# Makiato1999/HRI-EMO

Hardware: AMD Instinct MI355X
Metric: utterances/sec fwd+bwd, d=768 T_a=400 T_t=128 N_e=6 (higher is better)
Workload: dtype bf16; 1 GPU; FusionWithEmotionDecoder fwd+bwd (train mode, dropout 0.1), d=768 T_a=400 T_t=128 N_e=6 H=8, 2 fusion + 2 decoder layers, all-False masks (BASELINE cfg2); global_batch=64, batch_per_gpu=64, parallelism=dp1, grad_allreduce=none, launch=hipGraph replay, streams=2

## Files before the change

### hri-emo_amd/__init__.py

```python
from . import _lib
from .models.cross_modal_block_tacfn import CrossModalBlock, CrossModalTransformer
from .models.beta_gate_tacfn import BetaGate
from .models.emotion_decoder import EmotionDecoder, ExplainableDecoderLayer
from .models.fusion_with_emotion_decoder import FusionWithEmotionDecoder
from .models.mosei_fusion_with_emotion_decoder import MoseiFusionWithEmotionDecoder
from .models.fusion_classifier import FusionClassifier

from .dp import EvalStep
from ._ops import set_gemm_mode, gemm_mode, enable_fused_wgrad, set_precision, precision, set_varlen, varlen, set_varlen_maps, varlen_maps, set_mfma_maps, mfma_maps, set_ingest, ingest

__all__ = ["EvalStep", "set_gemm_mode", "gemm_mode", "enable_fused_wgrad", "set_precision", "precision", "set_varlen", "varlen", "set_varlen_maps", "varlen_maps", "set_mfma_maps", "mfma_maps", "set_ingest", "ingest", "CrossModalBlock", "CrossModalTransformer", "BetaGate", "EmotionDecoder", "ExplainableDecoderLayer",
           "FusionWithEmotionDecoder", "MoseiFusionWithEmotionDecoder", "FusionClassifier"]
```

### hri-emo_amd/_lib.py

```python
import ctypes
import os

_HERE = os.path.dirname(os.path.abspath(__file__))
LIB_PATH = os.environ.get("HRIEMO_LIB") or os.path.join(_HERE, "libhriemo.so")

_C = {"p": ctypes.c_void_p, "i": ctypes.c_int, "l": ctypes.c_long, "f": ctypes.c_float,
      "Q": ctypes.c_ulonglong, "I": ctypes.c_uint}

_SIGS = {
    "hriemo_gemm_bf16": ("iiiiiplplplipipliplp", "i"),
    "hriemo_gemm_force_config": ("i", "i"),
    "hriemo_gemm_debug_flags": ("i", "i"),
    "hriemo_gemm_colsum_rows": ("iiiii", "i"),
    "hriemo_gemm_plan": ("iiiiiilppp", "i"),
    "hriemo_gemm_bf16_group_tn": ("piip", "i"),
    "hriemo_gemm_bf16_split": ("iiiiiplplplpliiplp", "i"),
    "hriemo_gemm_bf16_colsum": ("iiiiiplplplplpp", "i"),
    "hriemo_mx8_scale_ld": ("i", "l"),
    "hriemo_quant_mx8": ("pliiiplplp", "i"),
    "hriemo_gemm_mx8": ("iiiplplplplplipiplp", "i"),
    "hriemo_gemm_mx8_q": ("iiiplplplplplpiplplp", "i"),
    "hriemo_gemm_mx8_force_config": ("i", "i"),
    "hriemo_attn_fwd": ("plplplplppiiiiifQpIipp", "i"),
    "hriemo_attn_fwd_q": ("plplplplppiiiiifQpIipplplp", "i"),
    "hriemo_attn_bwd": ("plplplplplplplplpppiiiiifQpIipppp", "i"),
    "hriemo_attn_fwd_varlen": ("plplplplpppiiiiifQpIipp", "i"),
    "hriemo_attn_fwd_q_varlen": ("plplplplpppiiiiifQpIipplpllp", "i"),
    "hriemo_attn_bwd_varlen": ("plplplplplplplplppppiiiiifQpIipppp", "i"),
    "hriemo_attn_mask_bytes": ("iiii", "l"),
    "hriemo_attn_bwd_single_pass": ("iiii", "i"),
    "hriemo_attn_bwd_single_pass_q": ("iiiii", "i"),
    "hriemo_attn_bwd_kv_colsum_rows": ("iiiii", "i"),
    "hriemo_attn_bwd_colsum_rows": ("iiii", "i"),
    "hriemo_attn_bwd_dq_colsum_rows": ("iiiii", "i"),
    "hriemo_attn_plan": ("iiiiiipppppp", "i"),
    "hriemo_split_bf16x3": ("pliipiip", "i"),
    "hriemo_attn_fwd_f32": ("plplplplppiiiiifQpIip", "i"),
    "hriemo_attn_probs_f32": ("plplpppiiiiifQpIip", "i"),
    "hriemo_add_ln_f32": ("ppppppiiffQpIlp", "i"),
    "hriemo_dropout_f32": ("ppliipfQpIlp", "i"),
    "hriemo_masked_mean_f32": ("pppiiip", "i"),
    "hriemo_gate_input_f32": ("pppiip", "i"),
    "hriemo_sigmoid_beta_f32": ("pppiip", "i"),
    "hriemo_fuse_f32": ("ppipippiiip", "i"),
    "hriemo_split3_f32": ("pliipiiplp", "i"),
    "hriemo_colsum_f32_workspace_bytes": ("ii", "l"),
    "hriemo_colsum_f32": ("pliiplpipp", "i"),
    "hriemo_add_ln_bwd_f32_workspace_bytes": ("ii", "l"),
    "hriemo_add_ln_bwd_f32": ("pppppppppiiiffQpIlpp", "i"),
    "hriemo_attn_bwd_f32": ("plplplplplppplplplpiiiiifQpIip", "i"),
    "hriemo_gate_dpre_f32": ("ppipipppiiip", "i"),
    "hriemo_gate_input_bwd_f32": ("pppppiip", "i"),
    "hriemo_gate_dy_f32": ("ppipppiiiip", "i"),
    "hriemo_rowdot_bwd_f32": ("ppppppiiip", "i"),
    "hriemo_attn_fwd_f32_varlen": ("plplplplpppiiiiifQpIip", "i"),
    "hriemo_attn_bwd_f32_varlen": ("plplplplplpppplplplpiiiiifQpIip", "i"),
    "hriemo_add_ln_f32_rows": ("ppppppiiffQpIlpp", "i"),
    "hriemo_add_ln_bwd_f32_rows": ("pppppppppiiiffQpIlppp", "i"),
    "hriemo_masked_mean_f32_packed": ("ppipiiip", "i"),
    "hriemo_fuse_f32_packed": ("pppiippiipppiiiip", "i"),
    "hriemo_gate_dpre_f32_packed": ("ppippiippiipppiiip", "i"),
    "hriemo_gate_dy_f32_packed": ("ppipippipiiiip", "i"),
    "hriemo_attn_probs": ("plplpppiiiiifQpIip", "i"),
    "hriemo_attn_probs_mfma": ("plplpppiiiiifQpIip", "i"),
    "hriemo_attn_probs_varlen": ("plplppppiiiiiiifQpIip", "i"),
    "hriemo_attn_probs_f32_varlen": ("plplppppiiiiiiifQpIip", "i"),
    "hriemo_add_ln_fwd": ("pppppppppiiffQpIlp", "i"),
    "hriemo_add_ln_fwd_mx8": ("pppppppppiiffQpIlpplp", "i"),
    "hriemo_add_ln_fwd_rows": ("pppppppppiiffQpIlpplpp", "i"),
    "hriemo_add_ln_bwd_rows": ("ppppppppppppiiifQpIlppp", "i"),
    "hriemo_add_ln_bwd_workspace_bytes": ("ii", "l"),
    "hriemo_add_ln_bwd": ("ppppppppppppiiifQpIlpp", "i"),
    "hriemo_colsum_workspace_bytes": ("ii", "l"),
    "hriemo_colsum_bf16": ("pliipipp", "i"),
    "hriemo_cast_f32_to_bf16": ("pplp", "i"),
    "hriemo_cast_bf16_to_f32": ("pplp", "i"),
    "hriemo_cast_f32_to_bf16_batch": ("pip", "i"),
    "hriemo_cast_copy_batch": ("pip", "i"),
    "hriemo_pack_rows": ("pppiiiipppp", "i"),
    "hriemo_unpack_rows": ("pppiiippp", "i"),
    "hriemo_ingest_rows": ("pilpiiiiipppplpp", "i"),
    "hriemo_seq_tables": ("ppiiiiippppppp", "i"),
    "hriemo_gather_rows": ("plppiplp", "i"),
    "hriemo_dropout_bf16": ("pplifQpIlp", "i"),
    "hriemo_gemm_ln_supported": ("i", "i"),
    "hriemo_gemm_ln_fwd": ("iiiplplppppppppppffQpIlpp", "i"),
    "hriemo_expand_rows": ("pppilp", "i"),
    "hriemo_seed_bump": ("pp", "i"),
    "hriemo_rowdot_fwd": ("pppppiip", "i"),
    "hriemo_rowdot_bwd": ("pppppppiiip", "i"),
    "hriemo_pool_chunks": ("i", "i"),
    "hriemo_ln_pool_fwd": ("pppppppppiiiifp", "i"),
    "hriemo_gate_input": ("ppppiiiipppp" + "p", "i"),
    "hriemo_sigmoid_beta": ("pppiip", "i"),
    "hriemo_fuse_fwd": ("ppppiiip", "i"),
    "hriemo_add_ln_bwd_partial_rows": ("ii", "i"),
    "hriemo_rowops_force_variant": ("i", "i"),
    "hriemo_colsum_partial_rows": ("ii", "i"),
    "hriemo_colreduce_batch": ("pipip", "i"),
    "hriemo_debug_hog": ("iipp", "i"),
    "hriemo_sumsq_f32": ("plpip", "i"),
    "hriemo_adamw_flat": ("pppplfffffifpp", "i"),
    "hriemo_optim_finalize": ("pippppp", "i"),
    "hriemo_adamw_flat_dev": ("pppplppp", "i"),
    "hriemo_grad_begin": ("plpp", "i"),
    "hriemo_optim_finalize_ctl": ("pipppppp", "i"),
    "hriemo_masked_mean_fwd": ("ppppiiip", "i"),
    "hriemo_rowsum_f32": ("ppilp", "i"),
    "hriemo_gate_input_pooled": ("pppiip", "i"),
    "hriemo_fusion_loss": ("ppppiiiffpppp", "i"),
    "hriemo_fusion_loss_ce": ("pppiiiffpppp", "i"),
    "hriemo_fusion_loss_n": ("ppppiiiffppppp", "i"),
    "hriemo_fusion_loss_ce_n": ("pppiiiffppppp", "i"),
    "hriemo_stats_update": ("ppppfpipiiippippp", "i"),
    "hriemo_predict_log": ("ppipiiipppipp", "i"),
    "hriemo_attn_log_plan": ("ppiipppp", "i"),
    "hriemo_attn_log_close": ("pp", "i"),
    "hriemo_attn_log_append": ("piippip", "i"),
    "hriemo_attn_probs_varlen_log": ("plplppppiiiiiiifQpIipip", "i"),
    "hriemo_attn_probs_varlen_log_fp32": ("plplppppiiiiiiifQpIipip", "i"),
    "hriemo_stats_counts": ("ppiippipp", "i"),
    "hriemo_stats_auc_tiles": ("i", "i"),
    "hriemo_stats_auc": ("ppiipppp", "i"),
    "hriemo_scalar_gate_dx":("pipippppiiip", "i"),
    "hriemo_fuse_bwd_dw": ("ppppiiip", "i"),
    "hriemo_gate_dpre": ("pippp" + "iip", "i"),
    "hriemo_gate_input_bwd": ("ppppppiip", "i"),
    "hriemo_ln_pool_bwd_chunks": ("i", "i"),
    "hriemo_ln_pool_pair_supported": ("i", "i"),
    "hriemo_ln_pool_fwd_pair": ("pppppppppi" * 2 + "iiifp", "i"),
    "hriemo_ln_pool_bwd_pair": ("pip" + "ppppppppppip" * 2 + "iiip", "i"),
    "hriemo_ln_pool_bwd_workspace_bytes": ("iii", "l"),
    "hriemo_ln_pool_bwd": ("pipipppppppppp" + "iiiipp", "i"),
    "hriemo_ln_pool_fwd_packed": ("pppiippppppipiiifp", "i"),
    "hriemo_ln_pool_fwd_packed_pair": ("pppiippppppi" * 2 + "piiifp", "i"),
    "hriemo_fuse_fwd_packed": ("pppppiiiip", "i"),
    "hriemo_fuse_fwd_packed_q": ("pppppiiiipplp", "i"),
    "hriemo_fuse_bwd_dw_packed": ("pppppiiiip", "i"),
    "hriemo_ln_pool_bwd_packed": ("ppipippppiipppppp" + "iiiipp", "i"),
    "hriemo_ln_pool_bwd_packed_pair": ("ppip" + "ppppiippppppip" * 2 + "iiip", "i"),
    "hriemo_prof_enable": ("i", "i"),
    "hriemo_prof_nclass": ("", "i"),
    "hriemo_prof_collect": ("ippp", "i"),
    "hriemo_abi_version": ("", "i"),
}

_lib = None


def lib():
    global _lib
    if _lib is None:
        if not os.path.exists(LIB_PATH):
            raise RuntimeError(
                f"{LIB_PATH} not found: build it with `make -C hri-emo_amd/csrc` (or __graft_entry__.build()). "
                "There is no CPU/eager fallback for this path.")
        L = ctypes.CDLL(LIB_PATH)
        for name, (args, res) in _SIGS.items():
            fn = getattr(L, name)
            fn.argtypes = [_C[c] for c in args]
            fn.restype = _C[res]
        L.hriemo_last_error.restype = ctypes.c_char_p
        L.hriemo_last_error.argtypes = []
        L.hriemo_prof_name.restype = ctypes.c_char_p
        L.hriemo_prof_name.argtypes = [ctypes.c_int]
        _lib = L
    return _lib


def call(name, *args):
    L = lib()
    rc = getattr(L, name)(*args)
    if rc != 0:
        raise RuntimeError(f"{name} failed ({rc}): {L.hriemo_last_error().decode()}")
```

### hri-emo_amd/_ops.py

```python
import itertools
import os as _os
import threading
from collections import namedtuple

import torch

from . import _lib

BF16 = torch.bfloat16
_EPS = 1e-5
_apply_tls = threading.local()


def _stream():
    return torch.cuda.current_stream().cuda_stream


def _p(t):
    return None if t is None else t.data_ptr()


def _require_fp32_master(p):
    if p.dtype != torch.float32:
        raise TypeError(f"hri_emo_amd: parameter of dtype {p.dtype}; keep the module's parameters in fp32 "
# ... 102 lines not shown
        t.record_stream(stream)
    return t


class TextBranch:

    def __init__(self, side, main):
        self.side, self.main = side, main

    def fork(self, *handed):
        if self.side is not None:
            fork(self.side, self.main)
            for x in handed:
                share(x, self.side)

    def run(self):
        return torch.cuda.stream(self.side)

    def join(self, *back):
        if self.side is not None:
            self.main.wait_stream(self.side)
            for x in back:
                share(x, self.main)


_site_counter = itertools.count(1)


def new_site_base():
    return next(_site_counter) * 4


_seed_words = {}
STEP_ID = 0


def begin_step():
    global STEP_ID
    STEP_ID += 1
    CTX.half_reports.clear()

WEIGHTS_EPOCH = 0


def bump_weights_epoch():
    global WEIGHTS_EPOCH
    WEIGHTS_EPOCH += 1


def seed_word(device):
    t = _seed_words.get(device.index)
    if t is None:
        t = torch.zeros(1, dtype=torch.int64, device=device)
        _seed_words[device.index] = t
    return t


DROP_LOG = None
_ones = {}


def one(device):
    t = _ones.get(device.index)
    if t is None:
        t = _ones[device.index] = torch.ones((), dtype=torch.float32, device=device)
    return t


def _is_one(g):
    t = _ones.get(g.device.index) if g.is_cuda else None
    return t is not None and g.data_ptr() == t.data_ptr() and g.dim() == 0


def bump_seed_word(device):
    _lib.call("hriemo_seed_bump", _p(seed_word(device)), _stream())


def next_seed(training):
    if not training:
        return 0
    return int(torch.randint(0, 2 ** 62, (1,)).item())


class Shadows:

    def __init__(self):
        self._d = {}

    def get(self, p):
        key = id(p)
        ent = self._d.get(key)
        ver = (p._version, p.data_ptr(), WEIGHTS_EPOCH)
        if (CTX.capturing and (ent is None or len(ent) < 3 or ent[2] != STEP_ID)) or ent is None or ent[0] != ver or ent[1].device != p.device:
            s = ent[1] if ent is not None and ent[1].device == p.device and ent[1].shape == p.shape else \
                torch.empty(p.shape, dtype=BF16, device=p.device)
            _require_gpu(p)
            _require_fp32_master(p)
            src = p.detach()
            if not src.is_contiguous():
                src = src.contiguous()
            _lib.call("hriemo_cast_f32_to_bf16", _p(src), _p(s), src.numel(), _stream())
            ent = (ver, s, STEP_ID)
            self._d[key] = ent
        return ent[1]

    def prefetch(self, params):
        for p in params:
            self.get(p)

    def stale(self, p):
        ent = self._d.get(id(p))
        ver = (p._version, p.data_ptr(), WEIGHTS_EPOCH)
        need = (CTX.capturing and (ent is None or len(ent) < 3 or ent[2] != STEP_ID)) or ent is None or ent[0] != ver or ent[1].device != p.device
        dst = ent[1] if ent is not None and ent[1].device == p.device and ent[1].shape == p.shape else None
        return need, dst, ver

    def get_cat(self, parts):
        key = ("cat",) + tuple((id(p), r0, r1) for p, r0, r1 in parts)
        ent = self._d.get(key)
        ver = tuple((p._version, p.data_ptr()) for p, _, _ in parts) + (WEIGHTS_EPOCH,)
        dev = parts[0][0].device
        if (CTX.capturing and (ent is None or ent[2] != STEP_ID)) or ent is None or ent[0] != ver or ent[1].device != dev:
            rows = sum(r1 - r0 for _, r0, r1 in parts)
            K = parts[0][0].shape[1]
            s = ent[1] if ent is not None and ent[1].device == dev else torch.empty((rows, K), dtype=BF16, device=dev)
            at = 0
            for p, r0, r1 in parts:
                _require_gpu(p)
                _require_fp32_master(p)
                src = p.detach()
                if not src.is_contiguous():
                    src = src.contiguous()
                _lib.call("hriemo_cast_f32_to_bf16", _p(src[r0:r1]), _p(s[at:at + (r1 - r0)]), (r1 - r0) * K, _stream())
                at += r1 - r0
            ent = (ver, s, STEP_ID)
            self._d[key] = ent
        return ent[1]

    def get_cat_wb(self, wparts, bparts):
        kw = ("cat",) + tuple((id(p), r0, r1) for p, r0, r1 in wparts)
        kb = ("catv",) + tuple((id(p), r0, r1) for p, r0, r1 in bparts)
        ew, eb = self._d.get(kw), self._d.get(kb)
        vw = tuple((p._version, p.data_ptr()) for p, _, _ in wparts) + (WEIGHTS_EPOCH,)
        vb = tuple((p._version, p.data_ptr()) for p, _, _ in bparts) + (WEIGHTS_EPOCH,)
        dev = wparts[0][0].device
        stale_w = (CTX.capturing and (ew is None or ew[2] != STEP_ID)) or ew is None or ew[0] != vw or ew[1].device != dev
        stale_b = (CTX.capturing and (eb is None or eb[2] != STEP_ID)) or eb is None or eb[0] != vb or eb[1].device != dev
        if not (stale_w or stale_b):
            return ew[1], eb[1]
        if not all(p.is_contiguous() for p, _, _ in wparts + bparts):
            return self.get_cat(wparts), self.get_cat_vec(bparts)
        K = wparts[0][0].shape[1]
        rows = sum(r1 - r0 for _, r0, r1 in wparts)
        nb = sum(r1 - r0 for _, r0, r1 in bparts)
        sw = ew[1] if ew is not None and ew[1].device == dev and ew[1].shape == (rows, K) else torch.empty((rows, K), dtype=BF16, device=dev)
        sb = eb[1] if eb is not None and eb[1].device == dev and eb[1].shape == (nb,) else torch.empty((nb,), dtype=torch.float32, device=dev)
        jobs, at = [], 0
        for p, r0, r1 in wparts:
            _require_gpu(p)
            _require_fp32_master(p)
            jobs.append((p.data_ptr() + r0 * K * 4, sw.data_ptr() + at * K * 2, (r1 - r0) * K, 0))
            at += r1 - r0
        at = 0
        for p, r0, r1 in bparts:
            _require_fp32_master(p)
            jobs.append((p.data_ptr() + r0 * 4, sb.data_ptr() + at * 4, r1 - r0, 1))
            at += r1 - r0
        if any(j[0] % 16 or j[1] % 16 for j in jobs):
            return self.get_cat(wparts), self.get_cat_vec(bparts)
        host = torch.tensor(jobs, dtype=torch.int64)
        _lib.call("hriemo_cast_copy_batch", host.data_ptr(), len(jobs), _stream())
        self._d[kw] = (vw, sw, STEP_ID)
        self._d[kb] = (vb, sb, STEP_ID)
        return sw, sb

    def get_cat_mx8(self, parts):
        key = ("catmx",) + tuple((id(p), r0, r1) for p, r0, r1 in parts)
        ent = self._d.get(key)
        ver = tuple((p._version, p.data_ptr()) for p, _, _ in parts) + (WEIGHTS_EPOCH,)
        if CTX.capturing or ent is None or ent[0] != ver:
            rows = sum(r1 - r0 for _, r0, r1 in parts)
            K = parts[0][0].shape[1]
            dev = parts[0][0].device
            L_ = _lib.lib()
            ld = L_.hriemo_mx8_scale_ld(rows)
            if ent is not None and ent[1][0].shape == (rows, K) and ent[1][0].device == dev:
                q, sc = ent[1]
            else:
                q = torch.empty((rows, K), dtype=torch.uint8, device=dev)
                sc = torch.zeros((K // 32, ld), dtype=torch.uint8, device=dev)
            at = 0
            for p, r0, r1 in parts:
                _require_gpu(p)
                _require_fp32_master(p)
                src = p.detach()
                if not src.is_contiguous():
                    src = src.contiguous()
                src = src[r0:r1]
                _lib.call("hriemo_quant_mx8", _p(src), src.stride(0), 1, r1 - r0, K, q.data_ptr() + at * K, K, sc.data_ptr() + at, ld,
                          _stream())
                at += r1 - r0
            ent = (ver, (q, sc))
            self._d[key] = ent
        return ent[1]

    def get_cat_vec(self, parts):
        key = ("catv",) + tuple((id(p), r0, r1) for p, r0, r1 in parts)
        ent = self._d.get(key)
        ver = tuple((p._version, p.data_ptr()) for p, _, _ in parts) + (WEIGHTS_EPOCH,)
        if (CTX.capturing and (ent is None or ent[2] != STEP_ID)) or ent is None or ent[0] != ver:
            v = torch.cat([p.detach()[r0:r1] for p, r0, r1 in parts])
            if ent is not None and ent[1].shape == v.shape and ent[1].device == v.device:
                ent[1].copy_(v)
                v = ent[1]
            ent = (ver, v, STEP_ID)
            self._d[key] = ent
        return ent[1]


FUSED_WGRAD = True


def enable_fused_wgrad(params, on=True):
    for p in params:
        p._hriemo_fused_grad = bool(on)


class GradSink:

    def __init__(self, params):
        self.params = params
        self.fused = FUSED_WGRAD and all(
            getattr(p, "_hriemo_fused_grad", False)
            and p.grad is not None and p.grad.dtype == torch.float32 and p.grad.is_contiguous()
            and p.grad.device == p.device and p.grad.shape == p.shape for p in params)
        if self.fused:
            for p in params:
                if hasattr(p, "_hriemo_grad_ready"):
                    p._hriemo_sink_managed = True

    def buf(self, p):
        return p.grad if self.fused else torch.empty(p.shape, dtype=torch.float32, device=p.device)

    def ret(self, t):
        return None if self.fused else t

    def done(self, skip=(), after_flush=()):
        if self.fused:
            for p in self.params:
                if any(p is q for q in skip):
                    continue
                hook = getattr(p, "_hriemo_grad_ready", None)
                if hook is not None:
                    if (p.dim() < 2 or any(p is q for q in after_flush)) and _small_dw.touches(p.grad):
                        _small_dw.add_hook(hook, p, True)
                    elif (p.dim() < 2 or any(p is q for q in after_flush)) and DEFER_REDUCE and _in_backward():
                        _deferred.add_hook(hook, p)
                    elif p.dim() >= 2 and _small_dw.touches(p.grad):
                        _small_dw.add_hook(hook, p)
                    else:
                        hook(p)


def prefetch_batch(pairs):
    jobs, upd = [], []
    for sh, p in pairs:
        need, dst, ver = sh.stale(p)
        if not need:
            continue
        _require_gpu(p)
        _require_fp32_master(p)
        if not p.is_contiguous() or p.data_ptr() % 16:
            sh.get(p)
            continue
        if dst is None:
            dst = torch.empty(p.shape, dtype=BF16, device=p.device)
        jobs.append((p.data_ptr(), dst.data_ptr(), p.numel()))
        upd.append((sh, id(p), ver, dst))
    if jobs:
        host = torch.tensor(jobs, dtype=torch.int64)
        _lib.call("hriemo_cast_f32_to_bf16_batch", host.data_ptr(), len(jobs), _stream())
        for sh, key, ver, dst in upd:
            sh._d[key] = (ver, dst, STEP_ID)


def padded_shadow(sh, p, kp):
    key = (id(p), "pad")
    ent = sh._d.get(key)
    ver = (p._version, p.data_ptr(), WEIGHTS_EPOCH)
    if CTX.capturing or ent is None or ent[0] != ver or ent[1].device != p.device:
        _require_gpu(p)
        _require_fp32_master(p)
        s_ = ent[1] if ent is not None and ent[1].device == p.device else \
            torch.zeros((p.shape[0], kp), dtype=BF16, device=p.device)
        s_[:, :p.shape[1]].copy_(p.detach())
        ent = (ver, s_)
        sh._d[key] = ent
    return ent[1]


def to_bf16(x):
    return x if x.dtype == BF16 else x.to(BF16)


def mask_u8(mask, B, L):
    if mask is None:
        return None
    if mask.shape != (B, L):
        raise ValueError(f"key_padding_mask shape {tuple(mask.shape)} != {(B, L)}")
    m = mask.contiguous()
    return m.view(torch.uint8) if m.dtype == torch.bool else m.to(torch.uint8)


def gemm(ta, tb, M, N, K, A, lda, B, ldb, C, ldc, c_f32=False, bias=None, epi=0, aux=None, ldaux=0, accumulate=False):
    ws = workspace(64 << 20, C.device) if c_f32 else None
    _lib.call("hriemo_gemm_bf16", ta, tb, M, N, K, _p(A), lda, _p(B), ldb, _p(C), ldc, int(c_f32), _p(bias), epi,
              _p(aux), ldaux, int(accumulate), _p(ws), ws.numel() * 4 if ws is not None else 0, _stream())


def linear_fwd(x, w16, bias, relu=False, out_f32=False):
    M, K = x.shape
    N = w16.shape[0]
    y = torch.empty((M, N), dtype=torch.float32 if out_f32 else BF16, device=x.device)
    gemm(0, 0, M, N, K, x, x.stride(0), w16, w16.stride(0), y, N, c_f32=out_f32, bias=bias, epi=1 if relu else 0)
    return y


def linear_dx(dy, w16, epi=0, aux=None):
    M, N = dy.shape
    K = w16.shape[1]
    dx = torch.empty((M, K), dtype=BF16, device=dy.device)
    gemm(0, 1, M, K, N, dy, dy.stride(0), w16, w16.stride(0), dx, K, epi=epi, aux=aux,
         ldaux=aux.stride(0) if aux is not None else 0)
    return dx


FOLD_FFN_BIAS = True


def fold_ffn_bias():
    return FOLD_FFN_BIAS


def linear_dx_masked_colsum(dy, w16, aux, bias_out, accumulate):
    M, N = dy.shape
    K = w16.shape[1]
    dx = torch.empty((M, K), dtype=BF16, device=dy.device)
    rows = _lib.lib().hriemo_gemm_colsum_rows(0, 1, M, K, N)
    part = torch.empty(rows * K, dtype=torch.float32, device=dy.device)
    _lib.call("hriemo_gemm_bf16_colsum", 0, 1, M, K, N, _p(dy), dy.stride(0), _p(w16), w16.stride(0), _p(dx), K, _p(aux), aux.stride(0),
              _p(part), _stream())
    if accumulate and DEFER_REDUCE and _in_backward():
        _deferred.add(part, K, rows, K, 1, [bias_out], True)
    else:
        red = _DeferredReduce()
        red.device = dy.device
        red.add(part, K, rows, K, 1, [bias_out], accumulate, schedule=False)
        red.flush()
    return dx


def linear_dw(dy, x, out, accumulate=False):
    M, N = dy.shape
    K = x.shape[1]
    if accumulate and M <= SMALL_DW_ROWS and _small_dw.enabled():
        _small_dw.add(dy, x, out)
# ... 1907 lines not shown
```

### hri-emo_amd/csrc/common.h

```cpp
#pragma once
#include <hip/hip_runtime.h>
#include <stdint.h>

typedef __bf16 bf16_t;
typedef __attribute__((ext_vector_type(2))) __bf16 bf16x2;
typedef __attribute__((ext_vector_type(4))) __bf16 bf16x4;
typedef __attribute__((ext_vector_type(8))) __bf16 bf16x8;
typedef __attribute__((ext_vector_type(4))) float f32x4;
typedef __attribute__((ext_vector_type(4))) short s16x4;

#define LDS_PTR(T) __attribute__((address_space(3))) T*
#define GLB_PTR(T) __attribute__((address_space(1))) T*

void hriemo_set_error(const char* fmt, ...);
#define HRIEMO_CHECK(cond, ...)            \
  do {                                     \
    if (!(cond)) {                         \
      hriemo_set_error(__VA_ARGS__);       \
      return 1;                            \
    }                                      \
  } while (0)
#define HRIEMO_LAUNCH_CHECK(name)                                         \
  do {                                                                    \
    hipError_t e__ = hipGetLastError();                                   \
// ... 19 lines not shown
  PackedSpan s;
  s.c0 = min(max(c0, 0), n_rows);
  s.len = max(min(min(c1, n_rows) - s.c0, cap), 0);
  return s;
}

__host__ __device__ __forceinline__ uint32_t fmix32(uint32_t x) {
  x ^= x >> 16; x *= 0x85ebca6bu; x ^= x >> 13; x *= 0xc2b2ae35u; x ^= x >> 16;
  return x;
}
__host__ __device__ __forceinline__ uint32_t site_key(uint64_t seed, uint32_t site, uint32_t c) {
  uint32_t k = fmix32((uint32_t)seed ^ 0x9e3779b9u);
  k = fmix32(k + (uint32_t)(seed >> 32) * 0x85ebca77u + site * 0x27d4eb2fu);
  return fmix32(k + c * 0x165667b1u);
}
#define DROP_CA 0x9e3779b1u
#define DROP_CB 0x85ebca77u
__host__ __device__ __forceinline__ uint32_t mul24(uint32_t a, uint32_t b) {
  return (a & 0xffffffu) * (b & 0xffffffu);
}
__host__ __device__ __forceinline__ uint32_t mix24(uint32_t x) {
  x ^= x >> 16; x = mul24(x, 0xB2AE35u); x ^= x >> 13; x = mul24(x, 0xEBCA6Bu); x ^= x >> 15;
  return x;
}
__host__ __device__ __forceinline__ uint32_t drop_base(uint32_t key, uint32_t a, uint32_t bp) {
  return key + a * DROP_CA + bp * DROP_CB;
}
__host__ __device__ __forceinline__ bool keep_lo(uint32_t x, uint32_t thr16) { return (x & 0xffffu) >= thr16; }
__host__ __device__ __forceinline__ bool keep_hi(uint32_t x, uint32_t thr16) { return (x >> 16) >= thr16; }
__host__ __device__ __forceinline__ bool keep16(uint32_t key, uint32_t a, uint32_t b, uint32_t thr16) {
  const uint32_t x = mix24(drop_base(key, a, b >> 1));
  return (b & 1u) ? keep_hi(x, thr16) : keep_lo(x, thr16);
}

struct DropCfg {
  uint64_t seed;
  uint32_t site;
  uint32_t thr16;
  float inv_keep;
};
__device__ __forceinline__ uint64_t eff_seed(uint64_t seed, const unsigned long long* seed_dev) {
  return seed + (seed_dev != nullptr ? (uint64_t)*seed_dev : 0ull);
}
static inline DropCfg make_drop(float p, uint64_t seed, uint32_t site) {
  DropCfg d;
  d.seed = seed; d.site = site;
  long t = (long)(p * 65536.0 + 0.5);
  if (t < 0) t = 0;
  if (t > 65535) t = 65535;
  d.thr16 = (uint32_t)t;
  d.inv_keep = (float)(1.0 / (1.0 - (double)t / 65536.0));
  return d;
}

__device__ __forceinline__ __attribute__((ext_vector_type(2))) int mx8_block(const float (&f)[8], int& e_out) {
  float amax = 0.f;
#pragma unroll
  for (int j = 0; j < 8; ++j) amax = fmaxf(amax, fabsf(f[j]));
  amax = fmaxf(amax, __shfl_xor(amax, 1));
  amax = fmaxf(amax, __shfl_xor(amax, 2));
  const unsigned ab = __float_as_uint(amax);
  int e = (int)(ab >> 23) - 8 + ((ab & 0x7fffffu) > 0x600000u ? 1 : 0);
  e = amax == 0.f ? 0 : (e < 1 ? 1 : (e > 253 ? 253 : e));
  const float inv = amax == 0.f ? 0.f : __uint_as_float((unsigned)(254 - e) << 23);
  int w0 = 0, w1 = 0;
  w0 = __builtin_amdgcn_cvt_pk_fp8_f32(f[0] * inv, f[1] * inv, w0, false);
  w0 = __builtin_amdgcn_cvt_pk_fp8_f32(f[2] * inv, f[3] * inv, w0, true);
  w1 = __builtin_amdgcn_cvt_pk_fp8_f32(f[4] * inv, f[5] * inv, w1, false);
  w1 = __builtin_amdgcn_cvt_pk_fp8_f32(f[6] * inv, f[7] * inv, w1, true);
  e_out = e;
  return (__attribute__((ext_vector_type(2))) int){w0, w1};
}

__device__ __forceinline__ void bf8_to_f32(const bf16x8& v, float* f) {
#pragma unroll
  for (int i = 0; i < 8; ++i) f[i] = (float)v[i];
}
__device__ __forceinline__ bf16x8 f32_to_bf8(const float* f) {
  bf16x8 v;
#pragma unroll
  for (int i = 0; i < 8; ++i) v[i] = (bf16_t)f[i];
  return v;
}
```

### hri-emo_amd/csrc/optim.hip

```cpp
#include "common.h"

enum { HY_LR = 0, HY_BETA1, HY_BETA2, HY_EPS, HY_WD, HY_MAX_NORM };
enum { ST_STEP = 0, ST_SKIP, ST_COEF, ST_STEP_SIZE, ST_ISB2, ST_DECAY, ST_GRAD_NORM, ST_SKIPPED };
enum { CTL_N_VALID = 0, CTL_FIRST, CTL_LAST };

template <bool HOLD>
__global__ __launch_bounds__(256) void optim_finalize_kernel(const float* __restrict__ partial, int nblocks, const float* __restrict__ hyper,
                                                             const float* __restrict__ grad_scale, const float* __restrict__ found_inf,
                                                             float* __restrict__ state, const int* __restrict__ ctl) {
  __shared__ float red[4];
  if (HOLD && ctl[CTL_LAST] == 0) {
    if (threadIdx.x == 0) state[ST_SKIP] = 1.f;
    return;
  }
  float s = 0.f;
  for (int i = threadIdx.x; i < nblocks; i += 256) s += partial[i];
  s = wave_sum(s);
  if ((threadIdx.x & 63) == 0) red[threadIdx.x >> 6] = s;
  __syncthreads();
  if (threadIdx.x != 0) return;
  const float sum = red[0] + red[1] + red[2] + red[3];
  const float gs = grad_scale != nullptr ? grad_scale[0] : 1.f;
  const float norm = sqrtf(sum) / gs;
  const bool finite = (__float_as_uint(norm) & 0x7f800000u) != 0x7f800000u;
  const bool skip = !finite || (found_inf != nullptr && !(found_inf[0] == 0.f));
  state[ST_GRAD_NORM] = norm;
  if (skip) {
    state[ST_SKIP] = 1.f;
    state[ST_SKIPPED] += 1.f;
    return;
  }
  const float lr = hyper[HY_LR], b1 = hyper[HY_BETA1], b2 = hyper[HY_BETA2], wd = hyper[HY_WD], max_norm = hyper[HY_MAX_NORM];
  const float step = state[ST_STEP] + 1.f;
  const float bc1 = 1.f - powf(b1, step), bc2 = 1.f - powf(b2, step);
  float coef = 1.f;
  if (max_norm > 0.f) coef = fminf(1.f, max_norm / (norm + 1e-6f));
  state[ST_STEP] = step;
  state[ST_SKIP] = 0.f;
  state[ST_COEF] = coef / gs;
  state[ST_STEP_SIZE] = lr / bc1;
  state[ST_ISB2] = 1.f / sqrtf(bc2);
  state[ST_DECAY] = 1.f - lr * wd;
}

__global__ __launch_bounds__(256) void adamw_flat_dev_kernel(float* __restrict__ p, const float* __restrict__ g, float* __restrict__ m,
                                                             float* __restrict__ v, long n, const float* __restrict__ hyper,
                                                             const float* __restrict__ state) {
  if (state[ST_SKIP] != 0.f) return;
  const float b1 = hyper[HY_BETA1], b2 = hyper[HY_BETA2], eps = hyper[HY_EPS];
  const float coef = state[ST_COEF], step = state[ST_STEP_SIZE], isb2 = state[ST_ISB2], decay = state[ST_DECAY];
  const long nv = n >> 2;
  for (long i = (long)blockIdx.x * 256 + threadIdx.x; i < nv; i += (long)gridDim.x * 256) {
    f32x4 pp = *(const f32x4*)(p + i * 4), mm = *(const f32x4*)(m + i * 4), vv = *(const f32x4*)(v + i * 4);
    const f32x4 gg = *(const f32x4*)(g + i * 4) * coef;
#pragma unroll
    for (int e = 0; e < 4; ++e) {
      pp[e] *= decay;
      mm[e] += (gg[e] - mm[e]) * (1.f - b1);
      vv[e] = vv[e] * b2 + gg[e] * gg[e] * (1.f - b2);
      pp[e] -= step * mm[e] / (sqrtf(vv[e]) * isb2 + eps);
    }
    *(f32x4*)(p + i * 4) = pp; *(f32x4*)(m + i * 4) = mm; *(f32x4*)(v + i * 4) = vv;
  }
}

__global__ __launch_bounds__(256) void grad_begin_kernel(float* __restrict__ flat, long n, const int* __restrict__ ctl) {
  if (ctl[CTL_FIRST] == 0) return;
  const long nv = n >> 2;
  const f32x4 zero = {0.f, 0.f, 0.f, 0.f};
  for (long i = (long)blockIdx.x * 256 + threadIdx.x; i < nv; i += (long)gridDim.x * 256) *(f32x4*)(flat + i * 4) = zero;
}

extern "C" int hriemo_grad_begin(float* flat, long n, const int* ctl, hipStream_t st) {
  HRIEMO_CHECK(flat != nullptr && n > 0 && n % 4 == 0, "grad_begin: n=%ld must be a positive multiple of 4", n);
  HRIEMO_CHECK(((uintptr_t)flat % 16) == 0, "grad_begin: unaligned buffer");
  HRIEMO_CHECK(ctl != nullptr && ((uintptr_t)ctl % 4) == 0, "grad_begin: ctl is the int32 step-control block in device memory");
  long gsz = (n / 4 + 255) / 256;
  if (gsz > 4096) gsz = 4096;
  hipLaunchKernelGGL(grad_begin_kernel, dim3((int)gsz), dim3(256), 0, st, flat, n, ctl);
  HRIEMO_LAUNCH_CHECK("grad_begin_kernel");
  return 0;
}

extern "C" int hriemo_optim_finalize(const float* partial, int nblocks, const float* hyper, const float* grad_scale, const float* found_inf,
                                     float* state, hipStream_t st) {
  HRIEMO_CHECK(partial != nullptr && hyper != nullptr && state != nullptr, "optim_finalize: partial, hyper and state are required");
  HRIEMO_CHECK(nblocks > 0 && nblocks <= 4096, "optim_finalize: nblocks=%d out of range (1..4096)", nblocks);
  hipLaunchKernelGGL(optim_finalize_kernel<false>, dim3(1), dim3(256), 0, st, partial, nblocks, hyper, grad_scale, found_inf, state,
                     (const int*)nullptr);
  HRIEMO_LAUNCH_CHECK("optim_finalize_kernel");
  return 0;
}

extern "C" int hriemo_optim_finalize_ctl(const float* partial, int nblocks, const float* hyper, const float* grad_scale,
                                         const float* found_inf, float* state, const int* ctl, hipStream_t st) {
  HRIEMO_CHECK(partial != nullptr && hyper != nullptr && state != nullptr, "optim_finalize_ctl: partial, hyper and state are required");
  HRIEMO_CHECK(nblocks > 0 && nblocks <= 4096, "optim_finalize_ctl: nblocks=%d out of range (1..4096)", nblocks);
  HRIEMO_CHECK(ctl != nullptr && ((uintptr_t)ctl % 4) == 0, "optim_finalize_ctl: ctl is the int32 step-control block in device memory");
  hipLaunchKernelGGL(optim_finalize_kernel<true>, dim3(1), dim3(256), 0, st, partial, nblocks, hyper, grad_scale, found_inf, state, ctl);
  HRIEMO_LAUNCH_CHECK("optim_finalize_kernel<hold>");
  return 0;
}

extern "C" int hriemo_adamw_flat_dev(float* p, const float* g, float* m, float* v, long n, const float* hyper, const float* state,
                                     hipStream_t st) {
  HRIEMO_CHECK(n > 0 && n % 4 == 0, "adamw_flat_dev: n=%ld must be a positive multiple of 4", n);
  HRIEMO_CHECK(((uintptr_t)p % 16) == 0 && ((uintptr_t)g % 16) == 0 && ((uintptr_t)m % 16) == 0 && ((uintptr_t)v % 16) == 0,
               "adamw_flat_dev: unaligned buffer");
  HRIEMO_CHECK(hyper != nullptr && state != nullptr, "adamw_flat_dev: hyper and state are required");
  long gsz = (n / 4 + 255) / 256;
  if (gsz > 4096) gsz = 4096;
  hipLaunchKernelGGL(adamw_flat_dev_kernel, dim3((int)gsz), dim3(256), 0, st, p, g, m, v, n, hyper, state);
  HRIEMO_LAUNCH_CHECK("adamw_flat_dev_kernel");
  return 0;
}
```

### hri-emo_amd/csrc/rowops.hip

```cpp
#include "common.h"
#include <string.h>
#include <stdlib.h>

#define EPS_DEFAULT 1e-5f

struct RowDrop { uint64_t seed; const unsigned long long* seed_dev; uint32_t site, thr16; float inv_keep; const long long* rowmap; };
static RowDrop row_drop(float p, uint64_t seed, const unsigned long long* seed_dev, uint32_t site) {
  DropCfg d = make_drop(p, seed, site);
  RowDrop r; r.seed = seed; r.seed_dev = seed_dev; r.site = site; r.thr16 = d.thr16; r.inv_keep = d.inv_keep; r.rowmap = nullptr;
  return r;
}
__device__ __forceinline__ uint32_t row_key(const RowDrop& dr) {
  return dr.thr16 != 0 ? site_key(eff_seed(dr.seed, dr.seed_dev), dr.site, 0u) : 0u;
}

template <int NCH>
__device__ __forceinline__ void block_colsum(float* lds_row, const float (&acc)[NCH][8], int nchunk, int lane, int wave, int nwave) {
  for (int w = 0; w < nwave; ++w) {
    if (wave == w) {
#pragma unroll
      for (int c = 0; c < NCH; ++c) {
        const int ch = lane + 64 * c;
        if (ch < nchunk) {
#pragma unroll
// ... 1241 lines not shown
  }
  HRIEMO_LAUNCH_CHECK("add_ln_bwd_kernel");
  hriemo_prof_end(HP_ROWOPS, st, ((dX ? 1.0 : 0.0) + (dG ? 1.0 : 0.0) + 2.0 + (X32 ? 2.0 : (X ? 1.0 : 0.0))) * M * d * 2);
  if (dgamma == nullptr) return 0;
  float* scratch = workspace + (long)nb * 3 * d;
  ReduceOut ro; ro.o[0] = dgamma; ro.o[1] = dbeta; ro.o[2] = dbias;
  launch_colreduce(workspace, (long)3 * d, nb, ro, d, dbias != nullptr ? 3 : 2, accumulate, scratch, st);
  HRIEMO_LAUNCH_CHECK("colreduce_kernel");
  return 0;
}

extern "C" int hriemo_add_ln_bwd(const void* dY, const void* G, const void* X, const float* X32, const float* gamma, const float* mean,
                                 const float* rstd, void* dX, void* dG, float* dgamma, float* dbeta, float* dbias, int accumulate,
                                 int M, int d, float p_drop, unsigned long long seed, const unsigned long long* seed_dev,
                                 unsigned site, long row_offset, float* workspace, hipStream_t st) {
  return add_ln_bwd_impl(dY, G, X, X32, gamma, mean, rstd, dX, dG, dgamma, dbeta, dbias, accumulate, M, d, p_drop, seed, seed_dev, site,
                         row_offset, workspace, nullptr, st);
}
extern "C" int hriemo_add_ln_bwd_rows(const void* dY, const void* G, const void* X, const float* X32, const float* gamma, const float* mean,
                                      const float* rstd, void* dX, void* dG, float* dgamma, float* dbeta, float* dbias, int accumulate,
                                      int M, int d, float p_drop, unsigned long long seed, const unsigned long long* seed_dev,
                                      unsigned site, long row_offset, float* workspace, const long long* row_index, hipStream_t st) {
  return add_ln_bwd_impl(dY, G, X, X32, gamma, mean, rstd, dX, dG, dgamma, dbeta, dbias, accumulate, M, d, p_drop, seed, seed_dev, site,
                         row_offset, workspace, row_index, st);
}

extern "C" int hriemo_add_ln_bwd_partial_rows(int M, int d) { (void)d; return row_grid(M, lnb_cap(d)); }

static int colsum_slices(int M, int N) {
  const int ncg = (N / 8 + 63) / 64;
  int slices = 2048 / ncg;
  if (slices > (M + 15) / 16) slices = (M + 15) / 16;
  if (slices < 1) slices = 1;
  return slices;
}
extern "C" long hriemo_colsum_workspace_bytes(int M, int N) { return ((long)colsum_slices(M, N) + 64) * N * 4; }

extern "C" int hriemo_colsum_bf16(const void* X, long ldx, int M, int N, float* out, int accumulate, float* workspace, hipStream_t st) {
  HRIEMO_CHECK(M > 0 && N > 0 && N % 8 == 0 && ldx % 8 == 0, "colsum: bad shape M=%d N=%d ld=%ld", M, N, ldx);
  HRIEMO_CHECK(workspace != nullptr, "colsum: workspace required");
  const int ncg = (N / 8 + 63) / 64;
  const int slices = colsum_slices(M, N);
  const int rps = (M + slices - 1) / slices;
  hipLaunchKernelGGL(colsum_partial_kernel, dim3(ncg, slices), dim3(64), 0, st, (const bf16_t*)X, ldx, M, N, rps, workspace);
  if (out == nullptr) { HRIEMO_LAUNCH_CHECK("colsum_partial_kernel"); return 0; }
  ReduceOut ro; ro.o[0] = out; ro.o[1] = ro.o[2] = nullptr;
  launch_colreduce(workspace, (long)N, slices, ro, N, 1, accumulate, workspace + (long)slices * N, st);
  HRIEMO_LAUNCH_CHECK("colsum");
  return 0;
}

extern "C" int hriemo_colsum_partial_rows(int M, int N) { return colsum_slices(M, N); }

struct JobChunk { long long v[48 * 8]; };
__global__ void upload_jobs_kernel(const JobChunk c, long long* __restrict__ dst, int n) {
  for (int i = threadIdx.x; i < n * 8; i += blockDim.x) dst[i] = c.v[i];
}

extern "C" int hriemo_colreduce_batch(const void* jobs_host, int njobs, void* jobs_dev, int nblocks, hipStream_t st) {
  HRIEMO_CHECK(jobs_host != nullptr && jobs_dev != nullptr && njobs > 0 && nblocks > 0, "colreduce_batch: empty job table");
  for (int j0 = 0; j0 < njobs; j0 += 48) {
    JobChunk c;
    const int n = njobs - j0 < 48 ? njobs - j0 : 48;
    memcpy(c.v, (const long long*)jobs_host + (long)j0 * 8, (size_t)n * 64);
    hipLaunchKernelGGL(upload_jobs_kernel, dim3(1), dim3(256), 0, st, c, (long long*)jobs_dev + (long)j0 * 8, n);
  }
  HRIEMO_LAUNCH_CHECK("upload_jobs_kernel");
  hriemo_prof_begin(HP_ROWOPS, st);
  hipLaunchKernelGGL(colreduce_batch_kernel, dim3(nblocks), dim3(256), 0, st, (const long long*)jobs_dev, njobs);
  HRIEMO_LAUNCH_CHECK("colreduce_batch_kernel");
  hriemo_prof_end(HP_ROWOPS, st, 0.0);
  return 0;
}

extern "C" int hriemo_cast_f32_to_bf16(const float* src, void* dst, long n, hipStream_t st) {
  HRIEMO_CHECK(n > 0 && ((uintptr_t)src % 16) == 0 && ((uintptr_t)dst % 16) == 0, "cast: empty or unaligned");
  long g = ((n >> 3) + 255) / 256;
  if (g > 4096) g = 4096;
  if (g < 1) g = 1;
  hipLaunchKernelGGL(cast_f32_bf16_kernel, dim3((int)g), dim3(256), 0, st, src, (bf16_t*)dst, n);
  HRIEMO_LAUNCH_CHECK("cast_f32_bf16_kernel");
  return 0;
}
struct CastJobs { const float* src[64]; void* dst[64]; long n[64]; int first[65]; int njobs; unsigned long long f32_copy; };
__global__ __launch_bounds__(256) void cast_f32_bf16_batch_kernel(const CastJobs J) {
  int j = 0;
  while (j + 1 < J.njobs && (int)blockIdx.x >= J.first[j + 1]) ++j;
  const long n = J.n[j], base = ((long)blockIdx.x - J.first[j]) * 2048 + (long)threadIdx.x * 8;
  const float* src = J.src[j];
  if ((J.f32_copy >> j) & 1ull) {
    float* dst = (float*)J.dst[j];
    if (base + 8 <= n) {
      *(f32x4*)(dst + base) = *(const f32x4*)(src + base);
      *(f32x4*)(dst + base + 4) = *(const f32x4*)(src + base + 4);
    } else {
      for (long e = base; e < n; ++e) dst[e] = src[e];
    }
    return;
  }
  bf16_t* dst = (bf16_t*)J.dst[j];
  if (base + 8 <= n) {
    const f32x4 a = *(const f32x4*)(src + base), b = *(const f32x4*)(src + base + 4);
    float f[8] = {a[0], a[1], a[2], a[3], b[0], b[1], b[2], b[3]};
    *(bf16x8*)(dst + base) = f32_to_bf8(f);
  } else {
    for (long e = base; e < n; ++e) dst[e] = (bf16_t)src[e];
  }
}
static int cast_batch_impl(const long long* h, int njobs, int rec, hipStream_t st) {
  for (int j0 = 0; j0 < njobs; j0 += 64) {
    CastJobs J;
    const int nj = njobs - j0 < 64 ? njobs - j0 : 64;
    int blocks = 0;
    J.f32_copy = 0ull;
    for (int j = 0; j < nj; ++j) {
      const long long* r = h + (long)(j0 + j) * rec;
      HRIEMO_CHECK(r[2] > 0 && (r[0] % 16) == 0 && (r[1] % 16) == 0, "cast_batch: job %d empty or unaligned", j0 + j);
      HRIEMO_CHECK(rec == 3 || r[3] == 0 || r[3] == 1, "cast_batch: job %d has kind %lld (0 = fp32 -> bf16, 1 = fp32 copy)", j0 + j, r[3]);
      J.src[j] = (const float*)r[0]; J.dst[j] = (void*)r[1]; J.n[j] = (long)r[2];
      if (rec == 4 && r[3] == 1) J.f32_copy |= 1ull << j;
      J.first[j] = blocks;
      blocks += (int)((r[2] + 2047) / 2048);
    }
    J.first[nj] = blocks; J.njobs = nj;
    hriemo_prof_begin(HP_ROWOPS, st);
    hipLaunchKernelGGL(cast_f32_bf16_batch_kernel, dim3(blocks), dim3(256), 0, st, J);
    HRIEMO_LAUNCH_CHECK("cast_f32_bf16_batch_kernel");
    hriemo_prof_end(HP_ROWOPS, st, 0.0);
  }
  return 0;
}
extern "C" int hriemo_cast_f32_to_bf16_batch(const void* jobs_host, int njobs, hipStream_t st) {
  HRIEMO_CHECK(jobs_host != nullptr && njobs > 0, "cast_batch: empty job table");
  return cast_batch_impl((const long long*)jobs_host, njobs, 3, st);
}
extern "C" int hriemo_cast_copy_batch(const void* jobs_host, int njobs, hipStream_t st) {
  HRIEMO_CHECK(jobs_host != nullptr && njobs > 0, "cast_copy_batch: empty job table");
  return cast_batch_impl((const long long*)jobs_host, njobs, 4, st);
}
extern "C" int hriemo_cast_bf16_to_f32(const void* src, float* dst, long n, hipStream_t st) {
  HRIEMO_CHECK(n > 0, "cast: empty");
  long g = (n + 255) / 256;
  if (g > 4096) g = 4096;
  hipLaunchKernelGGL(cast_bf16_f32_kernel, dim3((int)g), dim3(256), 0, st, (const bf16_t*)src, dst, n);
  HRIEMO_LAUNCH_CHECK("cast_bf16_f32_kernel");
  return 0;
}

extern "C" int hriemo_dropout_bf16(const void* X, void* Y, long M, int N, float p_drop, unsigned long long seed,
                                   const unsigned long long* seed_dev, unsigned site, long row_offset, hipStream_t st) {
  HRIEMO_CHECK(M > 0 && N > 0 && N % 8 == 0, "dropout: bad shape");
  RowDrop dr = row_drop(p_drop, seed, seed_dev, site);
  long g = (M * (N / 8) + 255) / 256;
  if (g > 4096) g = 4096;
  hipLaunchKernelGGL(dropout_kernel, dim3((int)g), dim3(256), 0, st, (const bf16_t*)X, (bf16_t*)Y, M, N, dr, row_offset);
  HRIEMO_LAUNCH_CHECK("dropout_kernel");
  return 0;
}

typedef __attribute__((ext_vector_type(4))) unsigned u32x4r;
__device__ __forceinline__ void copy_row16(const char* src, char* dst, int bytes, int lane) {
  for (int o = lane * 16; o < bytes; o += 64 * 16) *(u32x4r*)(dst + o) = src ? *(const u32x4r*)(src + o) : (u32x4r){0u, 0u, 0u, 0u};
}
__global__ __launch_bounds__(256) void pack_rows_kernel(const bf16_t* __restrict__ X16, const float* __restrict__ X32, const int* __restrict__ cu,
                                                        int B, int L, int d, int n_rows, bf16_t* __restrict__ P16, float* __restrict__ P32,
                                                        long long* __restrict__ rows) {
  const int lane = threadIdx.x & 63;
  const int r = blockIdx.x * 4 + (threadIdx.x >> 6);
  if (r >= n_rows) return;
  int lo = 0, hi = B;
  while (lo < hi) {
    const int mid = (lo + hi + 1) >> 1;
    if (cu[mid] <= r) lo = mid; else hi = mid - 1;
  }
  const int b = lo, l = r - cu[b];
  const bool real = b < B && l < L;
  const long src = (long)b * L + l;
  if (rows != nullptr && lane == 0) rows[r] = src;
  if (P16 != nullptr) copy_row16(real ? (const char*)(X16 + src * d) : nullptr, (char*)(P16 + (long)r * d), d * 2, lane);
  if (P32 != nullptr) copy_row16(real ? (const char*)(X32 + src * d) : nullptr, (char*)(P32 + (long)r * d), d * 4, lane);
}
__global__ __launch_bounds__(256) void unpack_rows_kernel(const bf16_t* __restrict__ P16, const float* __restrict__ P32, const int* __restrict__ cu,
                                                          int B, int L, int d, bf16_t* __restrict__ Y16, float* __restrict__ Y32) {
  const int lane = threadIdx.x & 63;
  const long row = (long)blockIdx.x * 4 + (threadIdx.x >> 6);
  if (row >= (long)B * L) return;
  const int b = (int)(row / L), l = (int)(row - (long)b * L);
  const int c0 = cu[b], len = cu[b + 1] - c0;
  const bool real = l < len;
  const long src = (long)c0 + l;
  if (Y16 != nullptr) copy_row16(real ? (const char*)(P16 + src * d) : nullptr, (char*)(Y16 + row * d), d * 2, lane);
  if (Y32 != nullptr) copy_row16(real ? (const char*)(P32 + src * d) : nullptr, (char*)(Y32 + row * d), d * 4, lane);
}
extern "C" int hriemo_pack_rows(const void* X16, const float* X32, const int* cu_seqlens, int B, int L, int d, int n_rows, void* P16,
                                float* P32, long long* row_index, hipStream_t st) {
  HRIEMO_CHECK(B > 0 && L > 0 && d > 0 && d % 8 == 0 && n_rows > 0 && cu_seqlens != nullptr, "pack_rows: bad shape (B=%d L=%d d=%d n_rows=%d)", B, L, d, n_rows);
  HRIEMO_CHECK((X16 == nullptr) == (P16 == nullptr) && (X32 == nullptr) == (P32 == nullptr), "pack_rows: source and destination of a tensor must both be given or both be NULL");
  HRIEMO_CHECK(((uintptr_t)X16 % 16) == 0 && ((uintptr_t)X32 % 16) == 0 && ((uintptr_t)P16 % 16) == 0 && ((uintptr_t)P32 % 16) == 0, "pack_rows: unaligned operand");
  hriemo_prof_begin(HP_ROWOPS, st);
  hipLaunchKernelGGL(pack_rows_kernel, dim3((n_rows + 3) / 4), dim3(256), 0, st, (const bf16_t*)X16, X32, cu_seqlens, B, L, d, n_rows, (bf16_t*)P16, P32, row_index);
  HRIEMO_LAUNCH_CHECK("pack_rows_kernel");
  hriemo_prof_end(HP_ROWOPS, st, (double)n_rows * d * ((X16 ? 4.0 : 0.0) + (X32 ? 8.0 : 0.0)));
  return 0;
}
extern "C" int hriemo_unpack_rows(const void* P16, const float* P32, const int* cu_seqlens, int B, int L, int d, void* Y16, float* Y32,
// ... 274 lines not shown
  for (int l = wave; l < L; l += 4) {
    const bool valid = mask == nullptr || mask[(long)b * L + l] == 0;
    if (lane == 0 && valid) c += 1.f;
    if (valid && ch < nchunk) {
      const bf16x8 v = *(const bf16x8*)(X + ((long)b * L + l) * d + ch * 8);
#pragma unroll
      for (int j = 0; j < 8; ++j) acc[j] += (float)v[j];
    }
  }
#pragma unroll
  for (int j = 0; j < 8; ++j) red[wave][lane][j] = acc[j];
  if (lane == 0) cred[wave] = c;
  __syncthreads();
  if (wave == 0) {
    const float n = fmaxf(cred[0] + cred[1] + cred[2] + cred[3], 1.f);
    if (ch < nchunk) {
#pragma unroll
      for (int j = 0; j < 8; ++j)
        pooled[(long)b * d + ch * 8 + j] = (red[0][lane][j] + red[1][lane][j] + red[2][lane][j] + red[3][lane][j]) / n;
    }
    if (lane == 0 && blockIdx.x == 0) cnt[b] = n;
  }
}

__global__ __launch_bounds__(256) void rowsum_f32_kernel(const float* __restrict__ x, float* __restrict__ out, long n) {
  __shared__ float red[4];
  const int b = blockIdx.x;
  float s = 0.f;
  for (long i = threadIdx.x; i < n; i += 256) s += x[(long)b * n + i];
  s = wave_sum(s);
  if ((threadIdx.x & 63) == 0) red[threadIdx.x >> 6] = s;
  __syncthreads();
  if (threadIdx.x == 0) out[b] = red[0] + red[1] + red[2] + red[3];
}

__global__ void scalar_gate_dx_kernel(const bf16_t* __restrict__ dH, int Lf, const float* __restrict__ beta, int is_a,
                                      const float* __restrict__ dpool, const float* __restrict__ cnt, const uint8_t* __restrict__ mask,
                                      bf16_t* __restrict__ dX, int B, int L, int d) {
  const int nch = d >> 3;
  const long nv = (long)B * L * nch;
  for (long v = (long)blockIdx.x * blockDim.x + threadIdx.x; v < nv; v += (long)gridDim.x * blockDim.x) {
    const int ch = (int)(v % nch);
    const long row = v / nch;
    const int b = (int)(row / L), l = (int)(row - (long)b * L);
    const float coef = is_a ? beta[b] : 1.f - beta[b];
    const bool valid = mask == nullptr || mask[row] == 0;
    const float ic = valid ? 1.f / cnt[b] : 0.f;
    float o[8];
#pragma unroll
    for (int j = 0; j < 8; ++j) o[j] = ic * dpool[(long)b * d + ch * 8 + j];
    if (l < Lf) {
      const bf16x8 g = *(const bf16x8*)(dH + ((long)b * Lf + l) * d + ch * 8);
#pragma unroll
      for (int j = 0; j < 8; ++j) o[j] += coef * (float)g[j];
    }
    *(bf16x8*)(dX + row * d + ch * 8) = f32_to_bf8(o);
  }
}

__global__ __launch_bounds__(256) void gate_input_pooled_kernel(const float* __restrict__ a_pool, const float* __restrict__ t_pool,
                                                                bf16_t* __restrict__ gin, int d) {
  const int b = blockIdx.x;
  bf16_t* g = gin + (long)b * 4 * d;
  for (int c = threadIdx.x; c < d; c += 256) {
    const float a = a_pool[(long)b * d + c], t = t_pool[(long)b * d + c];
    g[c] = (bf16_t)a; g[d + c] = (bf16_t)t; g[2 * d + c] = (bf16_t)fabsf(a - t); g[3 * d + c] = (bf16_t)(a * t);
  }
}

__global__ __launch_bounds__(256) void sumsq_f32_kernel(const float* __restrict__ x, long n, float* __restrict__ partial) {
  __shared__ float red[4];
  float s = 0.f;
  const long nv = n >> 2;
  for (long v = (long)blockIdx.x * 256 + threadIdx.x; v < nv; v += (long)gridDim.x * 256) {
    const f32x4 t = *(const f32x4*)(x + v * 4);
    s += t[0] * t[0] + t[1] * t[1] + t[2] * t[2] + t[3] * t[3];
  }
  s = wave_sum(s);
  if ((threadIdx.x & 63) == 0) red[threadIdx.x >> 6] = s;
  __syncthreads();
  if (threadIdx.x == 0) partial[blockIdx.x] = red[0] + red[1] + red[2] + red[3];
}

__global__ __launch_bounds__(256) void adamw_flat_kernel(float* __restrict__ p, const float* __restrict__ g, float* __restrict__ m,
                                                         float* __restrict__ v, long n, float lr, float b1, float b2, float eps,
                                                         float wd, float bc1, float bc2, float max_norm, const float* __restrict__ norm2) {
  float coef = 1.f;
  if (max_norm > 0.f) coef = fminf(1.f, max_norm / (sqrtf(norm2[0]) + 1e-6f));
  const float step = lr / bc1, isb2 = 1.f / sqrtf(bc2);
  const long nv = n >> 2;
  for (long i = (long)blockIdx.x * 256 + threadIdx.x; i < nv; i += (long)gridDim.x * 256) {
    f32x4 pp = *(const f32x4*)(p + i * 4), mm = *(const f32x4*)(m + i * 4), vv = *(const f32x4*)(v + i * 4);
    const f32x4 gg = *(const f32x4*)(g + i * 4) * coef;
#pragma unroll
    for (int e = 0; e < 4; ++e) {
      pp[e] *= 1.f - lr * wd;
      mm[e] += (gg[e] - mm[e]) * (1.f - b1);
      vv[e] = vv[e] * b2 + gg[e] * gg[e] * (1.f - b2);
      pp[e] -= step * mm[e] / (sqrtf(vv[e]) * isb2 + eps);
    }
    *(f32x4*)(p + i * 4) = pp; *(f32x4*)(m + i * 4) = mm; *(f32x4*)(v + i * 4) = vv;
  }
}

extern "C" int hriemo_pool_chunks(int L) { return (L + 31) / 32; }

extern "C" int hriemo_ln_pool_fwd(const void* X, const float* X32, const unsigned char* mask, const float* gamma, const float* beta, void* Yn,
                                  float* mean, float* rstd, float* partials, int B, int L, int Lkeep, int d, float eps,
                                  hipStream_t st) {
  if (check_rows(B * L, d)) return 1;
  HRIEMO_CHECK(Lkeep >= 0 && Lkeep <= L, "ln_pool_fwd: Lkeep=%d out of range (L=%d)", Lkeep, L);
  const int nc = (L + 31) / 32;
  hriemo_prof_begin(HP_ROWOPS, st);
#define CALL(N)                                                                                                                  \
  if ((N) <= 2)                                                                                                                  \
    hipLaunchKernelGGL((ln_pool_fwd_kernel<N, ((N) <= 2)>), dim3(nc, B), dim3(256), d * 4, st, (const bf16_t*)X, X32, mask, gamma, beta, (bf16_t*)Yn, mean, rstd, partials, L, Lkeep, d, eps); \
  else                                                                                                                           \
    hipLaunchKernelGGL((ln_pool_fwd_kernel<N, false>), dim3(nc, B), dim3(256), d * 4, st, (const bf16_t*)X, X32, mask, gamma, beta, (bf16_t*)Yn, mean, rstd, partials, L, Lkeep, d, eps)
  DISPATCH_NCH(d, CALL)
#undef CALL
  HRIEMO_LAUNCH_CHECK("ln_pool_fwd_kernel");
  hriemo_prof_end(HP_ROWOPS, st, ((double)B * L + (double)B * Lkeep) * d * 2);
  return 0;
}

extern "C" int hriemo_ln_pool_pair_supported(int d) { return d % 8 == 0 && d <= 1024 ? 1 : 0; }
extern "C" int hriemo_ln_pool_fwd_pair(const void* Xa, const float* Xa32, const unsigned char* mask_a, const float* gamma_a, const float* beta_a,
                                       void* Yna, float* mean_a, float* rstd_a, float* partials_a, int La,
                                       const void* Xt, const float* Xt32, const unsigned char* mask_t, const float* gamma_t, const float* beta_t,
                                       void* Ynt, float* mean_t, float* rstd_t, float* partials_t, int Lt,
                                       int B, int Lkeep, int d, float eps, hipStream_t st) {
  if (check_rows(B * La, d) || check_rows(B * Lt, d)) return 1;
  HRIEMO_CHECK(Lkeep >= 0 && Lkeep <= La && Lkeep <= Lt, "ln_pool_fwd_pair: Lkeep=%d out of range (La=%d, Lt=%d)", Lkeep, La, Lt);
  HRIEMO_CHECK(hriemo_ln_pool_pair_supported(d), "ln_pool_fwd_pair: d=%d (pairs are built for d <= 1024; use two hriemo_ln_pool_fwd calls)", d);
  PoolFwdPair p;
  p.s[0] = PoolFwdSide{(const bf16_t*)Xa, Xa32, mask_a, gamma_a, beta_a, (bf16_t*)Yna, mean_a, rstd_a, partials_a, La, Lkeep, (La + 31) / 32};
  p.s[1] = PoolFwdSide{(const bf16_t*)Xt, Xt32, mask_t, gamma_t, beta_t, (bf16_t*)Ynt, mean_t, rstd_t, partials_t, Lt, Lkeep, (Lt + 31) / 32};
  const int nc = p.s[0].nc + p.s[1].nc;
  hriemo_prof_begin(HP_ROWOPS, st);
  if (d <= 512) hipLaunchKernelGGL((ln_pool_fwd_pair_kernel<1, true>), dim3(nc, B), dim3(256), d * 4, st, p, d, eps);
  else hipLaunchKernelGGL((ln_pool_fwd_pair_kernel<2, true>), dim3(nc, B), dim3(256), d * 4, st, p, d, eps);
  HRIEMO_LAUNCH_CHECK("ln_pool_fwd_pair_kernel");
  hriemo_prof_end(HP_ROWOPS, st, ((double)B * (La + Lt) + 2.0 * B * Lkeep) * d * 2);
  return 0;
}

extern "C" int hriemo_gate_input(const float* partials_a, const float* partials_t, const unsigned char* mask_a,
                                 const unsigned char* mask_t, int B, int La, int Lt, int d, void* gate_in, float* a_pool,
                                 float* t_pool, float* cnt, hipStream_t st) {
  HRIEMO_CHECK(B > 0 && d > 0, "gate_input: empty");
  hipLaunchKernelGGL(gate_input_kernel, dim3(B), dim3(256), 0, st, partials_a, (La + 31) / 32, partials_t, (Lt + 31) / 32, mask_a,
                     mask_t, La, Lt, d, (bf16_t*)gate_in, a_pool, t_pool, cnt);
  HRIEMO_LAUNCH_CHECK("gate_input_kernel");
  return 0;
}

extern "C" int hriemo_sigmoid_beta(const float* pre, float* w, float* beta, int B, int d, hipStream_t st) {
  HRIEMO_CHECK(B > 0 && d > 0, "sigmoid_beta: empty");
  hipLaunchKernelGGL(sigmoid_beta_kernel, dim3(B), dim3(256), 0, st, pre, w, beta, d);
  HRIEMO_LAUNCH_CHECK("sigmoid_beta_kernel");
  return 0;
}

extern "C" int hriemo_masked_mean_fwd(const void* X, const unsigned char* mask, float* pooled, float* cnt, int B, int L, int d,
                                      hipStream_t st) {
  if (check_rows(B * L, d)) return 1;
  hriemo_prof_begin(HP_ROWOPS, st);
  hipLaunchKernelGGL(masked_mean_fwd_kernel, dim3((d / 8 + 63) / 64, B), dim3(256), 0, st, (const bf16_t*)X, mask, pooled, cnt, L, d);
  HRIEMO_LAUNCH_CHECK("masked_mean_fwd_kernel");
  hriemo_prof_end(HP_ROWOPS, st, 1.0 * B * L * d * 2);
  return 0;
}

extern "C" int hriemo_gate_input_pooled(const float* a_pool, const float* t_pool, void* gate_in, int B, int d, hipStream_t st) {
  HRIEMO_CHECK(B > 0 && d > 0, "gate_input_pooled: empty");
  hipLaunchKernelGGL(gate_input_pooled_kernel, dim3(B), dim3(256), 0, st, a_pool, t_pool, (bf16_t*)gate_in, d);
  HRIEMO_LAUNCH_CHECK("gate_input_pooled_kernel");
  return 0;
}

extern "C" int hriemo_rowsum_f32(const float* x, float* out, int B, long n, hipStream_t st) {
  HRIEMO_CHECK(B > 0 && n > 0, "rowsum_f32: empty problem");
  hipLaunchKernelGGL(rowsum_f32_kernel, dim3(B), dim3(256), 0, st, x, out, n);
  HRIEMO_LAUNCH_CHECK("rowsum_f32_kernel");
  return 0;
}

extern "C" int hriemo_scalar_gate_dx(const void* dH, int Lf, const float* beta, int is_a, const float* dpool, const float* cnt,
                                     const unsigned char* mask, void* dX, int B, int L, int d, hipStream_t st) {
  if (check_rows(B * L, d)) return 1;
  HRIEMO_CHECK(Lf >= 0 && Lf <= L, "scalar_gate_dx: Lf=%d out of range (L=%d)", Lf, L);
  long g = ((long)B * L * (d / 8) + 255) / 256;
  if (g > 8192) g = 8192;
  hriemo_prof_begin(HP_ROWOPS, st);
  hipLaunchKernelGGL(scalar_gate_dx_kernel, dim3((int)g), dim3(256), 0, st, (const bf16_t*)dH, Lf, beta, is_a, dpool, cnt, mask,
                     (bf16_t*)dX, B, L, d);
  HRIEMO_LAUNCH_CHECK("scalar_gate_dx_kernel");
  hriemo_prof_end(HP_ROWOPS, st, 2.0 * B * L * d * 2);
  return 0;
}

extern "C" int hriemo_sumsq_f32(const float* x, long n, float* partial, int nblocks, hipStream_t st) {
  HRIEMO_CHECK(n > 0 && n % 4 == 0 && nblocks > 0 && nblocks <= 4096, "sumsq_f32: n=%ld must be a positive multiple of 4, 0 < nblocks <= 4096", n);
  HRIEMO_CHECK(((uintptr_t)x % 16) == 0, "sumsq_f32: unaligned buffer");
  hipLaunchKernelGGL(sumsq_f32_kernel, dim3(nblocks), dim3(256), 0, st, x, n, partial);
  HRIEMO_LAUNCH_CHECK("sumsq_f32_kernel");
  return 0;
}

extern "C" int hriemo_adamw_flat(float* p, const float* g, float* m, float* v, long n, float lr, float beta1, float beta2, float eps,
                                 float weight_decay, int step, float max_norm, const float* norm2, hipStream_t st) {
  HRIEMO_CHECK(n > 0 && n % 4 == 0 && step >= 1, "adamw_flat: n=%ld must be a positive multiple of 4 and step >= 1", n);
  HRIEMO_CHECK(((uintptr_t)p % 16) == 0 && ((uintptr_t)g % 16) == 0 && ((uintptr_t)m % 16) == 0 && ((uintptr_t)v % 16) == 0, "adamw_flat: unaligned buffer");
  HRIEMO_CHECK(max_norm <= 0.f || norm2 != nullptr, "adamw_flat: clipping needs the squared gradient norm");
  const float bc1 = 1.f - powf(beta1, (float)step), bc2 = 1.f - powf(beta2, (float)step);
  long gsz = (n / 4 + 255) / 256;
  if (gsz > 4096) gsz = 4096;
  hipLaunchKernelGGL(adamw_flat_kernel, dim3((int)gsz), dim3(256), 0, st, p, g, m, v, n, lr, beta1, beta2, eps, weight_decay, bc1, bc2,
                     max_norm, norm2);
  HRIEMO_LAUNCH_CHECK("adamw_flat_kernel");
  return 0;
}

extern "C" int hriemo_fuse_fwd(const float* w, const void* A, const void* T, void* H, int B, int L, int d, hipStream_t st) {
  if (check_rows(B * L, d)) return 1;
  long g = ((long)B * L * (d / 8) + 255) / 256;
  if (g > 8192) g = 8192;
  hriemo_prof_begin(HP_ROWOPS, st);
  hipLaunchKernelGGL(fuse_fwd_kernel, dim3((int)g), dim3(256), 0, st, w, (const bf16_t*)A, (const bf16_t*)T, (bf16_t*)H, B, L, d);
  HRIEMO_LAUNCH_CHECK("fuse_fwd_kernel");
  hriemo_prof_end(HP_ROWOPS, st, 3.0 * B * L * d * 2);
  return 0;
}

extern "C" int hriemo_fuse_bwd_dw(const void* dH, const void* A, const void* T, float* partials, int B, int L, int d,
                                  hipStream_t st) {
  if (check_rows(B * L, d)) return 1;
  const int nc = (L + 31) / 32;
#define CALL(N) hipLaunchKernelGGL((fuse_bwd_dw_kernel<N>), dim3(nc, B), dim3(256), d * 4, st, (const bf16_t*)dH, (const bf16_t*)A, (const bf16_t*)T, partials, L, d)
  DISPATCH_NCH(d, CALL)
#undef CALL
  HRIEMO_LAUNCH_CHECK("fuse_bwd_dw_kernel");
  return 0;
}

extern "C" int hriemo_gate_dpre(const float* partials, int L, const float* dbeta, const float* w, void* dpre, int B, int d,
                                hipStream_t st) {
  HRIEMO_CHECK(B > 0 && d > 0, "gate_dpre: empty");
  hipLaunchKernelGGL(gate_dpre_kernel, dim3(B), dim3(256), 0, st, partials, (L + 31) / 32, dbeta, w, (bf16_t*)dpre, d);
  HRIEMO_LAUNCH_CHECK("gate_dpre_kernel");
  return 0;
}

extern "C" int hriemo_gate_input_bwd(const void* dgin, const float* a_pool, const float* t_pool, const float* cnt, float* da,
                                     float* dt, int B, int d, hipStream_t st) {
  HRIEMO_CHECK(B > 0 && d > 0, "gate_input_bwd: empty");
  hipLaunchKernelGGL(gate_input_bwd_kernel, dim3(B), dim3(256), 0, st, (const bf16_t*)dgin, a_pool, t_pool, cnt, da, dt, d);
  HRIEMO_LAUNCH_CHECK("gate_input_bwd_kernel");
  return 0;
}

extern "C" int hriemo_ln_pool_bwd_chunks(int L) { return (L + POOL_BWD_ROWS - 1) / POOL_BWD_ROWS; }
extern "C" long hriemo_ln_pool_bwd_workspace_bytes(int B, int L, int d) { return ((long)B * hriemo_ln_pool_bwd_chunks(L) * 2 * d + 64L * 2 * d) * 4; }

extern "C" int hriemo_ln_pool_bwd(const void* dH, int Lf, const float* w, int is_a, const float* dpool, const unsigned char* mask,
                                  const void* X, const float* X32, const float* gamma, const float* mean, const float* rstd, void* dX,
                                  float* dgamma, float* dbeta, int accumulate, int B, int L, int d, float* workspace, hipStream_t st) {
  if (check_rows(B * L, d)) return 1;
  HRIEMO_CHECK(workspace != nullptr && Lf <= L && (dgamma == nullptr) == (dbeta == nullptr), "ln_pool_bwd: bad arguments");
  const int nc = hriemo_ln_pool_bwd_chunks(L);
  hriemo_prof_begin(HP_ROWOPS, st);
#define CALL(N) hipLaunchKernelGGL((ln_pool_bwd_kernel<N>), dim3(nc, B), dim3(256), ((N) <= 2 ? 5 : 2) * d * 4, st, (const bf16_t*)dH, Lf, w, is_a, dpool, mask, (const bf16_t*)X, X32, gamma, mean, rstd, (bf16_t*)dX, workspace, L, d)
  DISPATCH_NCH(d, CALL)
#undef CALL
  HRIEMO_LAUNCH_CHECK("ln_pool_bwd_kernel");
  hriemo_prof_end(HP_ROWOPS, st, (2.0 * B * L + (double)B * Lf) * d * 2);
  if (dgamma == nullptr) return 0;
  float* scratch = workspace + (long)B * nc * 2 * d;
  ReduceOut ro; ro.o[0] = dgamma; ro.o[1] = dbeta; ro.o[2] = nullptr;
  launch_colreduce(workspace, (long)2 * d, B * nc, ro, d, 2, accumulate, scratch, st);
  HRIEMO_LAUNCH_CHECK("colreduce_kernel");
  return 0;
}

extern "C" int hriemo_ln_pool_bwd_pair(const void* dH, int Lf, const float* w,
                                       const float* dpool_a, const unsigned char* mask_a, const void* Xa, const float* Xa32, const float* gamma_a,
                                       const float* mean_a, const float* rstd_a, void* dXa, float* dgamma_a, float* dbeta_a, int La, float* workspace_a,
                                       const float* dpool_t, const unsigned char* mask_t, const void* Xt, const float* Xt32, const float* gamma_t,
                                       const float* mean_t, const float* rstd_t, void* dXt, float* dgamma_t, float* dbeta_t, int Lt, float* workspace_t,
                                       int accumulate, int B, int d, hipStream_t st) {
  if (check_rows(B * La, d) || check_rows(B * Lt, d)) return 1;
  HRIEMO_CHECK(workspace_a != nullptr && workspace_t != nullptr && workspace_a != workspace_t && Lf <= La && Lf <= Lt, "ln_pool_bwd_pair: bad arguments");
  HRIEMO_CHECK(hriemo_ln_pool_pair_supported(d), "ln_pool_bwd_pair: d=%d (pairs are built for d <= 1024; use two hriemo_ln_pool_bwd calls)", d);
  HRIEMO_CHECK((dgamma_a == nullptr) == (dbeta_a == nullptr) && (dgamma_t == nullptr) == (dbeta_t == nullptr) && (dgamma_a == nullptr) == (dgamma_t == nullptr),
               "ln_pool_bwd_pair: the four LayerNorm gradients come together or not at all");
  PoolBwdPair p;
  p.s[0] = PoolBwdSide{dpool_a, mask_a, (const bf16_t*)Xa, Xa32, gamma_a, mean_a, rstd_a, (bf16_t*)dXa, workspace_a, La, hriemo_ln_pool_bwd_chunks(La)};
  p.s[1] = PoolBwdSide{dpool_t, mask_t, (const bf16_t*)Xt, Xt32, gamma_t, mean_t, rstd_t, (bf16_t*)dXt, workspace_t, Lt, hriemo_ln_pool_bwd_chunks(Lt)};
  const int nc = p.s[0].nc + p.s[1].nc;
  hriemo_prof_begin(HP_ROWOPS, st);
  if (d <= 512) hipLaunchKernelGGL((ln_pool_bwd_pair_kernel<1>), dim3(nc, B), dim3(256), 5 * d * 4, st, (const bf16_t*)dH, Lf, w, p, d);
  else hipLaunchKernelGGL((ln_pool_bwd_pair_kernel<2>), dim3(nc, B), dim3(256), 5 * d * 4, st, (const bf16_t*)dH, Lf, w, p, d);
  HRIEMO_LAUNCH_CHECK("ln_pool_bwd_pair_kernel");
  hriemo_prof_end(HP_ROWOPS, st, (2.0 * B * (La + Lt) + 2.0 * B * Lf) * d * 2);
// ... 155 lines not shown
```

### hri-emo_amd/dp.py

```python
import collections
import itertools
import logging
import os

import torch
import torch.distributed as dist

log = logging.getLogger("hri_emo_amd.dp")

_VARLEN_BUCKETS = max(1, int(os.environ.get("HRIEMO_VARLEN_BUCKETS", "64")))
_VARLEN_MAX_GRAPHS = max(1, int(os.environ.get("HRIEMO_VARLEN_MAX_GRAPHS", "48")))


def bucket_rows(n, B, L):
    g = max(8, (B * L) // _VARLEN_BUCKETS // 8 * 8)
    g = min(g, L)
    return (n // g + 1) * g


def packed_tables(la, lt, B, La, Lt):
    key = (bucket_rows(sum(la), B, La), bucket_rows(sum(lt), B, Lt))
    cu = lambda lens, rows: list(itertools.accumulate(lens, initial=0)) + [rows]
    return key, cu(la, key[0]), cu(lt, key[1]), cu([min(x, y) for x, y in zip(la, lt)], key[1])

# ... 144 lines not shown
                    ctx.__enter__()
            else:
                for st in streams:
                    if st != cur:
                        cur.wait_stream(st)
        try:
            if self._snap is not None:
                self._snap[s:e].copy_(self.flat[s:e])
            if self.comm_dtype == torch.float32:
                self._works.append((dist.all_reduce(self.flat[s:e], op=dist.ReduceOp.SUM, group=self.group, async_op=True), None))
            else:
                if self._stage is None:
                    self._stage = torch.empty(self.flat.numel(), dtype=self.comm_dtype, device=self.flat.device)
                st = self._stage[s:e]
                st.copy_(self.flat[s:e])
                self._works.append((dist.all_reduce(st, op=dist.ReduceOp.SUM, group=self.group, async_op=True), (s, e)))
        finally:
            if ctx is not None:
                ctx.__exit__(None, None, None)

    def _on_grad(self, p, from_sink=False):
        if self.suspended or (getattr(p, "_hriemo_sink_managed", False) and not from_sink) or id(p) in self._reported:
            return
        self._reported.add(id(p))
        bi = self._bucket_of[id(p)]
        self._pending[bi] += 1
        if self._pending[bi] == self.buckets[bi][2] and not self._launched[bi]:
            self._launch(bi)

    def _on_grad_sink(self, p):
        self._on_grad(p, from_sink=True)

    def _rebind(self):
        for p in self.params:
            off, n = self._offsets[id(p)], p.numel()
            if p.grad is None or p.grad.data_ptr() != self.flat.data_ptr() + off * 4:
                p.grad = self.flat[off:off + n].view_as(p)

    def zero_grad(self):
        self.flat.zero_()
        self._rebind()

    def finish(self):
        if self.world > 1 or self.force_exchange:
            for bi in range(len(self.buckets)):
                if not self._launched[bi]:
                    self._launch(bi)
            for w, rng in self._works:
                w.wait()
                if rng is not None:
                    self.flat[rng[0]:rng[1]].copy_(self._stage[rng[0]:rng[1]])
            self._works = []
            self._pending = [0] * len(self.buckets)
            self._launched = [False] * len(self.buckets)
            self._reported = set()
            for p in self.params:
                p._hriemo_sink_managed = False
            if self.world > 1:
                self.flat.mul_(1.0 / self.world)

    def grad_norm(self):
        return self.flat.norm()


def shard_bounds(global_batch, rank, world):
    if global_batch % world != 0:
        raise ValueError(f"global batch {global_batch} is not divisible by world size {world}")
    per = global_batch // world
    return rank * per, (rank + 1) * per


def _in_step_context(fn):
    import functools

    @functools.wraps(fn)
    def wrapper(self, *a, **k):
        from . import _ops
        with _ops.use_context(self.ctx):
            return fn(self, *a, **k)
    return wrapper


class _GraphRecord:
    __slots__ = ("graph", "loss", "keep", "seqs", "out")

    def __init__(self, graph, loss, keep, seqs=None, out=None):
        self.graph, self.loss, self.keep, self.seqs, self.out = graph, loss, keep, seqs, out

    def release(self):
        from . import _ops
        self.graph = self.loss = self.keep = self.seqs = self.out = None
        _ops.GRAPHS_ALIVE -= 1
        if _ops.GRAPHS_ALIVE == 0:
            del _ops._ws_retired[:]


class _HostBlock:
    __slots__ = ("dev", "host", "copied")

    def __init__(self, values, device):
        self.dev = torch.tensor(values, dtype=torch.int32, device=device)
        self.host = torch.tensor(values, dtype=torch.int32, pin_memory=self.dev.is_cuda)
        self.copied = None

    def upload(self, values):
        if self.copied is not None:
            self.copied.synchronize()
        self.host.copy_(torch.tensor(values, dtype=torch.int32))
        self.dev.copy_(self.host, non_blocking=True)
        self.copied = torch.cuda.Event()
        self.copied.record()


class _RaggedFront:
    __slots__ = ("lens", "masks", "bool", "same_width", "partial", "accum", "ctl")

    def __init__(self, lens, masks, same_width, partial=False, accum=1, ctl=None):
        self.lens, self.masks, self.bool = lens, masks, tuple(m.view(torch.bool) for m in masks)
        self.same_width, self.partial, self.accum, self.ctl = same_width, bool(partial), int(accum), ctl


_MaskSeen = collections.namedtuple("_MaskSeen", "ident key cu masks")


class _PackedState:
    __slots__ = ("B", "La", "Lt", "cu_a", "cu_t", "cu_f", "graphs", "pool", "front")

    def __init__(self, B, La, Lt, device, front=None):
        self.B, self.La, self.Lt, self.front = B, La, Lt, front
        self.cu_a, self.cu_t, self.cu_f = (torch.zeros(B + 2, dtype=torch.int32, device=device) for _ in range(3))
        self.graphs = collections.OrderedDict()
        self.pool = None

    def __getitem__(self, name):
        return getattr(self, name)


def _load_ragged(pb, static, fill, la, lt, ctl=None):
    front = pb.front
    n_utt = len(la)
    la, lt, key, own = ghost_plan(la, lt, pb.B, pb.La, pb.Lt)
    fill(static, n_utt, own, key)
    front.lens.upload([la, lt])
    if front.ctl is not None:
        front.ctl.upload(ctl_words(n_utt, *(ctl if ctl is not None else (1, 1))))
    return key


def _caller_rows(rows_a, rows_t, y):
    def fill(static, n_utt, own, key):
        for src, rows, n, n_rows in ((static[0], rows_a, own[0], key[0]), (static[1], rows_t, own[1], key[1])):
            if rows.data_ptr() != src.data_ptr():
                src[:n].copy_(rows, non_blocking=True)
            src[n:n_rows].zero_()
        if y is not None and y.data_ptr() != static[4].data_ptr():
            static[4][:n_utt].copy_(y, non_blocking=True)
    return fill


class _StoreFeed:
    __slots__ = ("store", "version", "B", "pad", "stride", "block", "__weakref__")

    def __init__(self, store, B, pad, device):
        self.store, self.version, self.B, self.pad = store, store.version, int(B), (int(pad[0]), int(pad[1]))
        self.stride = 2 * self.B + 1
        self.block = _HostBlock([0] * (3 * self.stride), device)
        store._holders.add(self)

    def close(self):
        self.store._holders.discard(self)

    def batch(self, ids, partial, who):
        st = self.store
        if st.version != self.version:
            raise RuntimeError(f"{who}: the store changed since the capture (append): capture_store() again")
        ids = st.check_ids(ids)
        n = len(ids)
        if n > self.B:
            raise ValueError(f"{who}: a batch of {n} utterances; the captured step holds at most B = {self.B}")
        if n != self.B and not partial:
            raise ValueError(f"{who}: a batch of {n} utterances; the captured step holds B = {self.B} (drop the batch, run it with "
                             "use_graph(False), or capture with partial_batches=True)")
        return (ids,) + _store_batch(st, ids, self.pad, who)

    def fill(self, ids, targets=True):
        def fill(static, n_utt, own, key):
            self.block.upload(self.store.plan_words(ids, self.stride))
            self.store.gather_into(self.block.dev, self.stride, n_utt, static[0], key[0], static[1], key[1], static[4] if targets else None)
        return fill


def _store_batch(store, ids, pad, who):
    la, lt = [store.lengths_a[i] for i in ids], [store.lengths_t[i] for i in ids]
    for name, ls, L in (("audio", la, pad[0]), ("text", lt, pad[1])):
        bad = [v for v in ls if v < 1 or v > L]
        if bad:
            raise ValueError(f"{who}: {name} length {bad[0]} outside [1, {L}]")
    return la, lt


def _store_capture_facts(who, model, store, ids, pad_to):
    from .data import DeviceFeatureStore
    if not isinstance(store, DeviceFeatureStore):
        raise TypeError(f"{who}: store is a data.DeviceFeatureStore")
    ids = store.check_ids(ids)
    dev = next(model.parameters()).device
    if store.device != dev:
        raise ValueError(f"{who}: the store lives on {store.device}, the model on {dev}")
    La, Lt = (int(v) for v in (pad_to if pad_to is not None else store.pad_to))
    if Lt > La:
        raise RuntimeError(f"{who}: L_t={Lt} > L_a={La}: the gate fuses over the text length and needs L_a >= L_t")
    if not hasattr(model, "audio_proj") and store.widths[0] != store.widths[1]:
        raise ValueError(f"{who}: the store's rows differ in width {store.widths}")
    return ids, (La, Lt)


def _record_graph(dev, seqs, pool, warm, body, warmed=None, settle=0.0):
    from . import _ops
    side = DataParallelStep._capture_streams.get(dev.index)
    if side is None:
        side = DataParallelStep._capture_streams[dev.index] = torch.cuda.Stream(device=dev)
    side.wait_stream(torch.cuda.current_stream())
    _ops.CTX.seq_override = seqs
    try:
        with torch.cuda.stream(side):
            for _ in range(2):
                warm()
            if warmed is not None:
                warmed()
        torch.cuda.current_stream().wait_stream(side)
        torch.cuda.synchronize()
        if settle:
            import time
            time.sleep(settle)
        graph = torch.cuda.CUDAGraph()
        _ops.CTX.capturing = True
        _ops.CTX.capture_origin = side
        _ops.begin_step()
        try:
            kw = {"pool": pool} if pool is not None else {}
            with torch.cuda.graph(graph, stream=side, capture_error_mode="thread_local", **kw):
                out = body()
        finally:
            _ops.CTX.capturing = False
            _ops.CTX.capture_origin = None
    finally:
        _ops.CTX.seq_override = None
    _ops.GRAPHS_ALIVE += 1
    keep = _ops._deferred.keep + _ops._small_dw.keep
    _ops._deferred.keep, _ops._small_dw.keep = [], []
    return _GraphRecord(graph, out, keep, seqs)


class DataParallelStep:

    _capture_streams = {}

    def __init__(self, model, loss_fn, group=None, bucket_bytes=32 << 20, overlap=True, comm_dtype=torch.float32, force_exchange=False,
                 launch_from="notify", force_queue=None):
        self.model, self.loss_fn = model, loss_fn
        self.force_queue = force_queue
        self._exchange_in_graph = False
        self._replay = True
        self.rank = dist.get_rank(group) if dist.is_initialized() else 0
        self.world = dist.get_world_size(group) if dist.is_initialized() else 1
        self.buckets = GradBuckets(model.parameters(), bucket_bytes, group, overlap, comm_dtype, force_exchange, launch_from)
        from . import _ops
        self.ctx = _ops.StepContext()
        self._record = None
        self._pb = None
        self._static = None
        self._mask_seen = None
        self._optimizer = None
        self._micro = 0
        self._stats = None
        self._stats_scale = 1.0
        self._outputs = None
        self._feed = None

    @property
    def captured(self):
        return self._record is not None or (self._pb is not None and len(self._pb.graphs) > 0)

    @property
    def _replaying(self):
        return self._replay and self.captured

    @property
    def store(self):
        return None if self._feed is None else self._feed.store

    def set_global_batch(self, global_batch):
        lo, hi = shard_bounds(global_batch, self.rank, self.world)
        if hasattr(self.model, "set_batch_offset"):
            self.model.set_batch_offset(lo)
        return lo, hi

    def attach_stats(self, stats, loss_scale=1.0):
        if self.captured:
            raise RuntimeError("attach_stats() comes before capture() / capture_packed(): the update is part of the captured step "
                               "(release_graph() first to change it)")
        self._stats, self._stats_scale, self._outputs = stats, float(loss_scale), None

    def _update_stats(self):
        out, self._outputs = self._outputs, None
        if self._stats is not None and out is not None:
            logits, beta, y, loss, n_valid = out
            self._stats.update(logits, beta, y, loss, n_valid=n_valid, loss_scale=self._stats_scale)

    def _fwd_bwd(self, h_a, h_t, m_a, m_t, y, zero=True, scale=None, ragged=None):
        from . import _ops
        pb = self._pb
        front = pb.front if (pb is not None and ragged is None) else None
        if front is not None:
            seqs = _ops.CTX.seq_override
            if seqs is None:
                raise RuntimeError("DataParallelStep: after capture_packed() the static rows are fed by step_packed() only")
            _ops.seq_tables(front.lens.dev, pb.La, pb.Lt, rows=(seqs[0].N, seqs[1].N), cu=(pb.cu_a, pb.cu_t, pb.cu_f), masks=front.masks)
        b = self.buckets
        if self.force_queue is None:
            _ops.gemm_contended(bool(b._hooks) and not b.suspended and b.world > 1)
        else:
            _ops.gemm_contended(bool(self.force_queue), force=True)
        ctl = front.ctl.dev if (front is not None and front.ctl is not None) else None
        if ctl is not None and front.accum > 1:
            from . import _lib
            _lib.call("hriemo_grad_begin", self.buckets.flat.data_ptr(), self.buckets.flat.numel(), ctl.data_ptr(), _ops._stream())
            self.buckets._rebind()
        elif zero:
            self.buckets.zero_grad()
        if ragged is not None:
            logits, beta, _ = self.model.forward_packed(h_a, h_t, ragged[0], ragged[1], pad_to=ragged[2])
        elif front is not None:
            logits, beta, _ = self.model._forward_rows(h_a, h_t, tuple(seqs), front.bool, (pb.La, pb.Lt))
        else:
            logits, beta, _ = self.model(h_a, h_t, m_a, m_t)
        if ctl is not None and front.partial:
            loss = self.loss_fn(logits, beta, y, n_valid=ctl[:1])
        else:
            loss = self.loss_fn(logits, beta, y)
        if self._stats is not None:
            self._outputs = (logits.detach(), None if beta is None else beta.detach(), y, loss.detach(),
                             ctl[:1] if (ctl is not None and front.partial) else None)
        if scale is not None:
            loss = loss * scale
        if loss.is_cuda and scale is None:
            loss.backward(gradient=_ops.one(loss.device))
        else:
            loss.backward()
        return loss.detach()

    @_in_step_context
    def step_accumulated(self, micro_batches, pad_to=None):
        from . import _ops
        k = len(micro_batches)
        was = self.buckets.suspended
        total = None
        for i, mb in enumerate(micro_batches):
            self.buckets.suspended = True if i + 1 < k else was
            if pad_to is not None:
                ra, rt, la, lt, y = mb
# ... 78 lines not shown
        from . import _ops
        dev = next(self.model.parameters()).device
        _ops._require_gpu(next(self.model.parameters()))
        self._begin_capture(entry, optimizer, collectives, packed=True)
        self._micro = 0
        B, (La, Lt) = len(la), pad
        cap_a, cap_t = bucket_rows(B * La, B, La), bucket_rows(B * Lt, B, Lt)
        src_a = torch.zeros(cap_a, widths[0], dtype=dtype, device=dev)
        src_t = torch.zeros(cap_t, widths[1], dtype=dtype, device=dev)
        self._static = [src_a, src_t, None, None, y_static]
        masks = tuple(torch.ones(B, L, dtype=torch.uint8, device=dev) for L in (La, Lt, Lt))
        ctl = _HostBlock(ctl_words(B, 1, 1), dev) if (partial_batches or grad_accum > 1) else None
        front = _RaggedFront(_HostBlock([[1] * B] * 2, dev), masks, not hasattr(self.model, "audio_proj"), partial_batches, grad_accum, ctl)
        self._pb = _PackedState(B, La, Lt, dev, front)
        try:
            if make_feed is not None:
                self._feed = make_feed(dev)
            self._packed_graph(load())
        except BaseException:
            self.release_graph()
            raise
        self._end_capture()

    @_in_step_context
    def capture_store(self, store, ids, pad_to=None, optimizer=None, collectives=False, partial_batches=False, grad_accum=1):
        self._check_ragged_capture("capture_store", partial_batches, grad_accum)
        ids, pad = _store_capture_facts("capture_store", self.model, store, ids, pad_to)
        B = len(ids)
        la, lt = _store_batch(store, ids, pad, "capture_store")
        dev = next(self.model.parameters()).device
        y_static = torch.zeros((B,) + tuple(store.y.shape[1:]), dtype=store.y.dtype, device=dev)
        self._capture_ragged("capture_store", store.widths, store.dtype, y_static, la, lt, pad, lambda: self._load_store(ids, la, lt), optimizer,
                             collectives, partial_batches, grad_accum, make_feed=lambda d: _StoreFeed(store, B, pad, d))

    @_in_step_context
    def step_store(self, ids):
        feed = self._feed
        if feed is None or self._pb is None or self._pb.front is None:
            raise RuntimeError("step_store needs capture_store() first")
        ids, la, lt = feed.batch(ids, self._pb.front.partial or not self._replaying, "step_store")
        if self._replaying:
            return self._replay_ragged(lambda ctl: self._load_store(ids, la, lt, ctl=ctl))
        rows_a, _, rows_t, _, y = feed.store.fetch(ids)
        return self._eager_ragged(rows_a, rows_t, la, lt, y)

    @_in_step_context
    def step_packed(self, rows_a, rows_t, lengths_a, lengths_t, y):
        from . import _ops
        pb = self._pb
        front = pb.front if pb is not None else None
        if front is None:
            raise RuntimeError("step_packed needs capture_packed() first")
        B, pad = pb.B, (pb.La, pb.Lt)
        la, lt, _ = _ops.packed_lengths(rows_a, rows_t, lengths_a, lengths_t, pad, same_width=front.same_width)
        if self._replaying:
            n = len(la)
            if n != B and not front.partial:
                raise ValueError(f"step_packed: a batch of {n} utterances; the captured step holds B = {B} (drop the batch, run it "
                                 "with use_graph(False), or capture with partial_batches=True)")
            if n > B:
                raise ValueError(f"step_packed: a batch of {n} utterances; the captured step holds at most B = {B}")
            for name, rows, src in (("rows_a", rows_a, self._static[0]), ("rows_t", rows_t, self._static[1])):
                if rows.shape[1] != src.shape[1] or rows.dtype != src.dtype:
                    raise ValueError(f"step_packed: {name} of width {rows.shape[1]} / {rows.dtype}; captured with width {src.shape[1]} / {src.dtype}")
            want = (n,) + tuple(self._static[4].shape[1:])
            if tuple(y.shape) != want:
                raise ValueError(f"step_packed: targets of shape {tuple(y.shape)}; captured with {tuple(self._static[4].shape)}"
                                 + (f", this batch needs {want}" if n != B else ""))
            return self._replay_ragged(lambda ctl: self._load_packed(rows_a, rows_t, la, lt, y, ctl=ctl))
        return self._eager_ragged(rows_a, rows_t, la, lt, y)

    def _load_packed(self, rows_a, rows_t, la, lt, y, ctl=None):
        return _load_ragged(self._pb, self._static, _caller_rows(rows_a, rows_t, y), la, lt, ctl)

    def _load_store(self, ids, la, lt, ctl=None):
        return _load_ragged(self._pb, self._static, self._feed.fill(ids), la, lt, ctl)

    def _replay_ragged(self, load):
        first, last = micro_flags(self._micro, self._pb.front.accum)
        if self._optimizer is not None and last:
            self._optimizer._upload_hyper()
        key = load((first, last))
        rec = self._packed_graph(key)
        rec.graph.replay()
        self._micro = 0 if last else self._micro + 1
        if last:
            self._after_replay()
        return rec.loss

    def _eager_ragged(self, rows_a, rows_t, la, lt, y):
        pb = self._pb
        first, last = micro_flags(self._micro, pb.front.accum)
        dev = self._static[0].device
        was = self.buckets.suspended
        if not last:
            self.buckets.suspended = True
        try:
            loss = self._fwd_bwd(rows_a.to(dev, non_blocking=True), rows_t.to(dev, non_blocking=True), None, None, y.to(dev, non_blocking=True),
                                 zero=first, ragged=(la, lt, (pb.La, pb.Lt)))
        finally:
            self.buckets.suspended = was
        self._update_stats()
        self._micro = 0 if last else self._micro + 1
        if last:
            self.buckets.finish()
            if self._optimizer is not None:
                self._optimizer.step()
        return loss

    @property
    def micro_step(self):
        return self._micro

    @_in_step_context
    def flush_accumulated(self):
        n = self._micro
        if n == 0:
            return 0
        self._micro = 0
        if not self._exchange_in_graph or not self._replaying:
            self.buckets.finish()
        if self._optimizer is not None:
            self._optimizer.step()
        return n

    def _packed_key(self, m_a, m_t, lengths):
        pb = self._pb
        la, lt = mask_lengths(m_a, m_t, lengths, pb.B, pb.La, pb.Lt)
        key, *tables = packed_tables(la, lt, pb.B, pb.La, pb.Lt)
        for buf, cu in zip((pb.cu_a, pb.cu_t, pb.cu_f), tables):
            buf.copy_(torch.tensor(cu, dtype=torch.int32))
        return key

    def _packed_graph(self, key):
        from . import _ops
        pb = self._pb
        rec = pb.graphs.get(key)
        if rec is None:
            rng = torch.get_rng_state() if self.captured else None
            while len(pb.graphs) >= _VARLEN_MAX_GRAPHS:
                old_key, old = pb.graphs.popitem(last=False)
                torch.cuda.synchronize()
                old.release()
                log.info("packed step: released the graph of bucket %s (cap %d)", old_key, _VARLEN_MAX_GRAPHS)
            seqs = (_ops.seq_bucket(pb.cu_a, pb.B, pb.La, key[0]), _ops.seq_bucket(pb.cu_t, pb.B, pb.Lt, key[1]),
                    _ops.seq_bucket_fused(pb.cu_f, pb.B, min(pb.La, pb.Lt), key[1]))
            front = pb.front
            held = self.buckets.flat.clone() if (front is not None and front.accum > 1 and self._micro > 0) else None
            try:
                rec = pb.graphs[key] = self._capture_graph(seqs)
            finally:
                if rng is not None:
                    torch.set_rng_state(rng)
                if held is not None:
                    self.buckets.flat.copy_(held)
            log.info("packed step: captured the graph of bucket (audio rows, text rows) = %s (%d alive)", key, len(pb.graphs))
        else:
            pb.graphs.move_to_end(key)
        return rec

    def _capture_graph(self, seqs):
        from . import _ops
        collectives = self._exchange_in_graph

        def warm():
            self._fwd_bwd(*self._static)
            if collectives:
                self.buckets.finish()

        def warmed():
            self._outputs = None

        def body():
            _ops.bump_seed_word(self._static[0].device)
            loss = self._fwd_bwd(*self._static)
            self._update_stats()
            if collectives:
                self.buckets.finish()
            if self._optimizer is not None:
                front = self._pb.front if self._pb is not None else None
                ctl = front.ctl.dev if (front is not None and front.accum > 1) else None
                self._optimizer._enqueue(ctl=ctl)
            return loss

        if seqs is not None and self._pb.pool is None:
            self._pb.pool = torch.cuda.graph_pool_handle()
        return _record_graph(self._static[0].device, seqs, self._pb.pool if seqs is not None else None, warm, body, warmed,
                             settle=0.25 if collectives else 0.0)

    def release_graph(self):
        if self.captured:
            torch.cuda.synchronize()
            for rec in ([self._record] if self._record is not None else self._pb.graphs.values()):
                rec.release()
            self._record = self._pb = self._optimizer = None
        if self._feed is not None:
            self._feed.close()
            self._feed = None

    def use_graph(self, on):
        self._replay = bool(on) and self.captured
        self.buckets.suspended = self._replay

    def _after_replay(self):
        if not self._exchange_in_graph:
            self.buckets.finish()
        if self._optimizer is not None:
            from . import _ops
            _ops.bump_weights_epoch()
            self._optimizer._opt_called = True

    @_in_step_context
    def step(self, h_a, h_t, m_a, m_t, y, lengths=None):
        if self._replaying:
            pb = self._pb
            if self._optimizer is not None:
                self._optimizer._upload_hyper()
            if pb is not None and pb.front is not None:
                raise RuntimeError("DataParallelStep: this step was captured by capture_packed(); feed it with step_packed()")
            if pb is not None:
                if m_a is None or m_t is None:
                    raise RuntimeError("DataParallelStep (packed mode): both padding masks are needed")
                ident = (m_a.data_ptr(), m_a._version, m_t.data_ptr(), m_t._version)
                seen = self._mask_seen
                if lengths is None and seen is not None and seen.ident == ident:
                    key = seen.key
                    for buf, saved in zip((pb.cu_a, pb.cu_t, pb.cu_f), seen.cu):
                        buf.copy_(saved)
                else:
                    key = self._packed_key(m_a, m_t, lengths)
                    self._mask_seen = _MaskSeen(ident, key, (pb.cu_a.clone(), pb.cu_t.clone(), pb.cu_f.clone()), (m_a, m_t))
            for s, t in zip(self._static, (h_a, h_t, m_a, m_t, y)):
                if s is not None and t is not None and s.data_ptr() != t.data_ptr():
                    s.copy_(t)
            rec = self._packed_graph(key) if pb is not None else self._record
            rec.graph.replay()
            self._after_replay()
            return rec.loss
        loss = self._fwd_bwd(h_a, h_t, m_a, m_t, y)
        self._update_stats()
        self.buckets.finish()
        if self._optimizer is not None:
            self._optimizer.step()
        return loss


def _mode_switches():
    from . import _ops
    return (("precision", _ops.precision()), ("gemm_mode", _ops.gemm_mode()), ("PACKED_TAIL", bool(_ops.PACKED_TAIL)),
            ("PACKED_TAIL_FP32", bool(_ops.PACKED_TAIL_FP32)), ("PACKED_TAIL_MX8", bool(_ops.PACKED_TAIL_MX8)), ("ingest", _ops.ingest()))


class EvalStep:

    def __init__(self, model, loss_fn=None, stats=None, log=None, max_graphs=None, attn_log=None):
        from . import _ops
        if max_graphs is not None and int(max_graphs) < 1:
            raise ValueError("EvalStep: max_graphs is a positive integer (or None)")
        self.model, self.loss_fn, self.stats, self.log, self.attn_log = model, loss_fn, stats, log, attn_log
        self.max_graphs = None if max_graphs is None else int(max_graphs)
        self.ctx = _ops.StepContext()
        self._pb = None
        self._static = None
        self._modes = None
        self._feed = None
        self._replay = True

    @property
    def captured(self):
        return self._pb is not None and len(self._pb.graphs) > 0

    @property
    def _replaying(self):
        return self._replay and self.captured

    @property
    def store(self):
        return None if self._feed is None else self._feed.store

    def use_graph(self, on):
        self._replay = bool(on) and self.captured

    def release_graph(self):
        if self.captured:
            torch.cuda.synchronize()
            for rec in self._pb.graphs.values():
                rec.release()
        self._pb = self._static = self._modes = None
        if self._feed is not None:
            self._feed.close()
            self._feed = None

    def _switches(self):
        from . import _ops
        if self.attn_log is None:
            return _mode_switches()
        return _mode_switches() + (("varlen_maps", _ops.varlen_maps()), ("mfma_maps", _ops.mfma_maps()))

    @_in_step_context
    def capture_packed(self, rows_a, rows_t, lengths_a, lengths_t, y=None, pad_to=None):
        from . import _ops
        if not hasattr(self.model, "_forward_rows"):
            raise TypeError("EvalStep.capture_packed: the model has no forward_packed entry")
        if self.loss_fn is not None and y is not None and not _accepts_n_valid(self.loss_fn):
            raise TypeError("EvalStep.capture_packed: loss_fn takes no n_valid= keyword -- the ghost utterances of a short batch must "
                            "stay out of the loss (hri_emo_amd.train's losses accept it)")
        if self.stats is not None and (self.loss_fn is None or y is None):
            raise ValueError("EvalStep.capture_packed: statistics need a loss_fn and targets (prediction-only graphs feed the log)")
        same_width = not hasattr(self.model, "audio_proj")
        la, lt, pad = _ops.packed_lengths(rows_a, rows_t, lengths_a, lengths_t, pad_to, same_width=same_width)
        if pad_to is None:
            raise ValueError("EvalStep.capture_packed: pad_to=(L_a, L_t) is required")
        dev = next(self.model.parameters()).device
        _ops._require_gpu(next(self.model.parameters()))
        B = len(la)
        if y is not None and y.shape[0] != B:
            raise ValueError(f"EvalStep.capture_packed: targets of shape {tuple(y.shape)} for {B} utterances")
        self._check_attn_log("capture_packed", pad)
        self._capture_ragged((rows_a.shape[1], rows_t.shape[1]), rows_a.dtype, None if y is None else y.to(dev, copy=True), la, lt, pad,
                             lambda: _caller_rows(rows_a, rows_t, y))

    def _check_attn_log(self, entry, pad):
        from . import _ops
        if self.attn_log is not None:
            if not _ops.varlen_maps():
                raise ValueError(f"EvalStep.{entry}: attention maps of packed rows need set_varlen_maps(True)")
            why = self.attn_log.mismatch(self.model, pad)
            if why is not None:
                raise ValueError(f"EvalStep.{entry}: the attention log does not fit: {why}")

    def _capture_ragged(self, widths, dtype, y_static, la, lt, pad, make_fill, make_feed=None):
        dev = next(self.model.parameters()).device
        self.release_graph()
        B, (La, Lt) = len(la), pad
        cap_a, cap_t = bucket_rows(B * La, B, La), bucket_rows(B * Lt, B, Lt)
        src_a = torch.zeros(cap_a, widths[0], dtype=dtype, device=dev)
        src_t = torch.zeros(cap_t, widths[1], dtype=dtype, device=dev)
        self._static = [src_a, src_t, None, None, y_static]
        masks = tuple(torch.ones(B, L, dtype=torch.uint8, device=dev) for L in (La, Lt, Lt))
        front = _RaggedFront(_HostBlock([[1] * B] * 2, dev), masks, not hasattr(self.model, "audio_proj"), partial=True, accum=1,
                             ctl=_HostBlock(ctl_words(B, 1, 1), dev))
        self._pb = _PackedState(B, La, Lt, dev, front)
        self._modes = self._switches()
        self._replay = True
        try:
            if make_feed is not None:
                self._feed = make_feed(dev)
            self._packed_graph(_load_ragged(self._pb, self._static, make_fill(), la, lt))
        except BaseException:
            self.release_graph()
            raise

    @_in_step_context
    def capture_store(self, store, ids, pad_to=None):
        from . import _ops
        if not hasattr(self.model, "_forward_rows"):
            raise TypeError("EvalStep.capture_store: the model has no forward_packed entry")
        targets = self.loss_fn is not None
        if targets and not _accepts_n_valid(self.loss_fn):
            raise TypeError("EvalStep.capture_store: loss_fn takes no n_valid= keyword -- the ghost utterances of a short batch must "
                            "stay out of the loss (hri_emo_amd.train's losses accept it)")
        if self.stats is not None and not targets:
            raise ValueError("EvalStep.capture_store: statistics need a loss_fn (prediction-only graphs feed the log)")
        ids, pad = _store_capture_facts("EvalStep.capture_store", self.model, store, ids, pad_to)
        B = len(ids)
        la, lt = _store_batch(store, ids, pad, "EvalStep.capture_store")
        dev = next(self.model.parameters()).device
        _ops._require_gpu(next(self.model.parameters()))
        self._check_attn_log("capture_store", pad)
        y_static = torch.zeros((B,) + tuple(store.y.shape[1:]), dtype=store.y.dtype, device=dev) if targets else None
        self._capture_ragged(store.widths, store.dtype, y_static, la, lt, pad, lambda: self._feed.fill(ids, targets),
                             make_feed=lambda d: _StoreFeed(store, B, pad, d))

    @_in_step_context
    def eval_store(self, ids):
        pb, feed = self._pb, self._feed
        if pb is None or feed is None:
            raise RuntimeError("eval_store needs capture_store() first")
        ids, la, lt = feed.batch(ids, True, "eval_store")
        targets = self._static[4] is not None
        if not self._replaying:
            rows_a, _, rows_t, _, y = feed.store.fetch(ids)
            return self._eval_eager(rows_a, rows_t, la, lt, y if targets else None)
        self._check_modes("eval_store", "capture_store")
        rec = self._packed_graph(_load_ragged(pb, self._static, feed.fill(ids, targets), la, lt))
        rec.graph.replay()
        logits, beta, z = rec.out
        n = len(ids)
        return logits[:n], beta[:n], z[:n], rec.loss

    def _pass(self, record):
        from . import _ops
        pb = self._pb
        front = pb.front
        seqs = _ops.CTX.seq_override
        y = self._static[4]
        with torch.no_grad():
            _ops.seq_tables(front.lens.dev, pb.La, pb.Lt, rows=(seqs[0].N, seqs[1].N), cu=(pb.cu_a, pb.cu_t, pb.cu_f), masks=front.masks)
            n_valid = front.ctl.dev[:1]
            if self.attn_log is not None:
                self.attn_log.plan(front.lens.dev, n_valid, pb.B, record=record)
                logits, beta, z = self.model._forward_rows(self._static[0], self._static[1], tuple(seqs), front.bool, (pb.La, pb.Lt),
                                                           attn_log=self.attn_log)
            else:
                logits, beta, z = self.model._forward_rows(self._static[0], self._static[1], tuple(seqs), front.bool, (pb.La, pb.Lt))
            loss = self.loss_fn(logits, beta, y, n_valid=n_valid) if (self.loss_fn is not None and y is not None) else None
            if record and self.stats is not None:
                self.stats.update(logits, beta, y, loss, n_valid=n_valid)
            if record and self.log is not None:
                self.log.update(logits, beta, n_valid=n_valid)
        return logits, beta, z, loss

    def _packed_graph(self, key):
        from . import _ops
        pb = self._pb
        rec = pb.graphs.get(key)
        if rec is not None:
            pb.graphs.move_to_end(key)
            return rec
        rng = torch.get_rng_state() if self.captured else None
        cap = self.max_graphs if self.max_graphs is not None else _VARLEN_MAX_GRAPHS
        while len(pb.graphs) >= cap:
            old_key, old = pb.graphs.popitem(last=False)
            torch.cuda.synchronize()
            old.release()
            log.info("eval step: released the graph of bucket %s (cap %d)", old_key, cap)
        seqs = (_ops.seq_bucket(pb.cu_a, pb.B, pb.La, key[0]), _ops.seq_bucket(pb.cu_t, pb.B, pb.Lt, key[1]),
                _ops.seq_bucket_fused(pb.cu_f, pb.B, min(pb.La, pb.Lt), key[1]))
        if pb.pool is None:
            pb.pool = torch.cuda.graph_pool_handle()
        was = self.model.training
        self.model.eval()
        try:
            rec = _record_graph(self._static[0].device, seqs, pb.pool, lambda: self._pass(False), lambda: self._pass(True))
        finally:
            self.model.train(was)
            if rng is not None:
                torch.set_rng_state(rng)
        rec.out, rec.loss = rec.loss[:3], rec.loss[3]
        pb.graphs[key] = rec
        log.info("eval step: captured the graph of bucket (audio rows, text rows) = %s (%d alive)", key, len(pb.graphs))
        return rec

    def _check_modes(self, entry="eval_packed", capture="capture_packed"):
        for (name, then), (_, now) in zip(self._modes, self._switches()):
            if then != now:
                raise RuntimeError(f"EvalStep.{entry}: the step was captured with {name} = {then!r}; it is {now!r} now -- "
                                   f"{capture}() again under the new setting, or switch back")

    @_in_step_context
    def eval_packed(self, rows_a, rows_t, lengths_a, lengths_t, y=None):
        from . import _ops
        pb = self._pb
        if pb is None:
            raise RuntimeError("eval_packed needs capture_packed() first")
        front = pb.front
        la, lt, _ = _ops.packed_lengths(rows_a, rows_t, lengths_a, lengths_t, (pb.La, pb.Lt), same_width=front.same_width)
        n = len(la)
        if not self._replaying:
            return self._eval_eager(rows_a, rows_t, la, lt, y)
        self._check_modes()
        if n > pb.B:
            raise ValueError(f"eval_packed: a batch of {n} utterances; the captured step holds at most B = {pb.B}")
        for name, rows, src in (("rows_a", rows_a, self._static[0]), ("rows_t", rows_t, self._static[1])):
            if rows.shape[1] != src.shape[1] or rows.dtype != src.dtype:
                raise ValueError(f"eval_packed: {name} of width {rows.shape[1]} / {rows.dtype}; captured with width {src.shape[1]} / {src.dtype}")
        sy = self._static[4]
        if sy is None and y is not None:
            raise ValueError("eval_packed: targets given, but the step was captured without (prediction-only graphs)")
        if sy is not None and y is None:
            raise ValueError("eval_packed: the step was captured with targets; this batch has none")
        if sy is not None:
            want = (n,) + tuple(sy.shape[1:])
            if tuple(y.shape) != want:
                raise ValueError(f"eval_packed: targets of shape {tuple(y.shape)}; captured with {tuple(sy.shape)}"
                                 + (f", this batch needs {want}" if n != pb.B else ""))
        rec = self._packed_graph(_load_ragged(pb, self._static, _caller_rows(rows_a, rows_t, y), la, lt))
        rec.graph.replay()
        logits, beta, z = rec.out
        return logits[:n], beta[:n], z[:n], rec.loss

    def _eval_eager(self, rows_a, rows_t, la, lt, y):
        pb = self._pb
        dev = self._static[0].device
        was = self.model.training
        self.model.eval()
        try:
            with torch.no_grad():
                extra = {} if self.attn_log is None else {"attn_log": self.attn_log}
                logits, beta, z = self.model.forward_packed(rows_a.to(dev, non_blocking=True), rows_t.to(dev, non_blocking=True), la, lt,
                                                            pad_to=(pb.La, pb.Lt), **extra)
                loss = None
                if self.loss_fn is not None and y is not None:
                    y = y.to(dev, non_blocking=True)
                    loss = self.loss_fn(logits, beta, y)
                    if self.stats is not None:
                        self.stats.update(logits, beta, y, loss)
                if self.log is not None:
                    self.log.update(logits, beta)
        finally:
            self.model.train(was)
        return logits, beta, z, loss
```

### hri-emo_amd/optim.py

```python
import torch

from . import _lib
from . import _ops
from ._ops import _p, _stream, _require_gpu


class FusedClipAdamW:
    def __init__(self, buckets, lr=1e-4, betas=(0.9, 0.999), eps=1e-8, weight_decay=1e-2, max_norm=5.0):
        self.buckets = buckets
        flat_g = buckets.flat
        _require_gpu(flat_g)
        self.lr, self.betas, self.eps, self.wd, self.max_norm = lr, betas, eps, weight_decay, max_norm
        self.flat_p = torch.zeros_like(flat_g)
        self.m = torch.zeros_like(flat_g)
        self.v = torch.zeros_like(flat_g)
        with torch.no_grad():
            for p in buckets.params:
                off, n = buckets._offsets[id(p)], p.numel()
                view = self.flat_p[off:off + n].view_as(p)
                view.copy_(p.data)
                p.data = view
        self.nblocks = 1024
        self._partial = torch.empty(self.nblocks, dtype=torch.float32, device=flat_g.device)
        self._norm2 = torch.zeros(1, dtype=torch.float32, device=flat_g.device)
        self.steps = 0

    @torch.no_grad()
    def step(self):
        g = self.buckets.flat
        n = g.numel()
        st = _stream()
        self.steps += 1
        _lib.call("hriemo_sumsq_f32", _p(g), n, _p(self._partial), self.nblocks, st)
        _lib.call("hriemo_rowsum_f32", _p(self._partial), _p(self._norm2), 1, self.nblocks, st)
        _lib.call("hriemo_adamw_flat", _p(self.flat_p), _p(g), _p(self.m), _p(self.v), n, self.lr, self.betas[0], self.betas[1],
                  self.eps, self.wd, self.steps, self.max_norm if self.max_norm else 0.0, _p(self._norm2), st)
        _ops.bump_weights_epoch()
        return self._norm2.sqrt()


class DeviceAdamW(torch.optim.Optimizer):

    _step_supports_amp_scaling = True

    def __init__(self, buckets, lr=1e-4, betas=(0.9, 0.999), eps=1e-8, weight_decay=1e-2, max_norm=5.0):
        flat_g = buckets.flat
        _require_gpu(flat_g)
        if lr < 0 or eps < 0 or weight_decay < 0 or not 0 <= betas[0] < 1 or not 0 <= betas[1] < 1:
            raise ValueError("DeviceAdamW: lr, eps, weight_decay >= 0 and betas in [0, 1) are required")
        self.buckets = buckets
        dev = flat_g.device
        self.flat_p = torch.zeros_like(flat_g)
        self.m = torch.zeros_like(flat_g)
        self.v = torch.zeros_like(flat_g)
        self.nblocks = 1024
        self._partial = torch.zeros(self.nblocks, dtype=torch.float32, device=dev)
        self._hyper = torch.zeros(8, dtype=torch.float32, device=dev)
        self._state = torch.zeros(8, dtype=torch.float32, device=dev)
        self._hyper_host = None
        defaults = dict(lr=lr, betas=tuple(betas), eps=eps, weight_decay=weight_decay, amsgrad=False, maximize=False, foreach=None,
                        capturable=False, differentiable=False, fused=None, decoupled_weight_decay=True, max_norm=max_norm)
        super().__init__(list(buckets.params), defaults)
        with torch.no_grad():
            for p in buckets.params:
                off, n = buckets._offsets[id(p)], p.numel()
                view = self.flat_p[off:off + n].view_as(p)
                view.copy_(p.data)
                p.data = view
                self.state[p] = {"step": self._state[0], "exp_avg": self.m[off:off + n].view_as(p),
                                 "exp_avg_sq": self.v[off:off + n].view_as(p)}
        self.grad_norm, self.device_step, self.skipped = self._state[6], self._state[0], self._state[7]

    def add_param_group(self, param_group):
        if self.param_groups:
            raise RuntimeError("DeviceAdamW updates ONE flat buffer laid out like its GradBuckets: it has exactly one param group")
        super().add_param_group(param_group)

    def _upload_hyper(self):
        g = self.param_groups[0]
        if g["amsgrad"] or g["maximize"]:
            raise RuntimeError("DeviceAdamW: amsgrad / maximize are not built; there is no fallback to torch.optim.AdamW")
        mn = g["max_norm"]
        img = (float(g["lr"]), float(g["betas"][0]), float(g["betas"][1]), float(g["eps"]), float(g["weight_decay"]),
               float(mn) if mn else 0.0, 0.0, 0.0)
        if img != self._hyper_host:
            self._hyper.copy_(torch.tensor(img, dtype=torch.float32).pin_memory(), non_blocking=True)
            self._hyper_host = img

    def _enqueue(self, grad_scale=None, found_inf=None, ctl=None):
        g = self.buckets.flat
        n = g.numel()
        st = _stream()
        _lib.call("hriemo_sumsq_f32", _p(g), n, _p(self._partial), self.nblocks, st)
        if ctl is None:
            _lib.call("hriemo_optim_finalize", _p(self._partial), self.nblocks, _p(self._hyper), _p(grad_scale), _p(found_inf),
                      _p(self._state), st)
        else:
            _lib.call("hriemo_optim_finalize_ctl", _p(self._partial), self.nblocks, _p(self._hyper), _p(grad_scale), _p(found_inf),
                      _p(self._state), _p(ctl), st)
        _lib.call("hriemo_adamw_flat_dev", _p(self.flat_p), _p(g), _p(self.m), _p(self.v), n, _p(self._hyper), _p(self._state), st)

    def _amp_word(self, name):
        t = getattr(self, name, None)
        if t is None:
            return None
        if not (isinstance(t, torch.Tensor) and t.is_cuda and t.dtype == torch.float32 and t.numel() == 1):
            raise RuntimeError(f"DeviceAdamW: {name} must be one fp32 value on the GPU (torch.amp.GradScaler's), got {t!r}")
        return t

    @torch.no_grad()
    def step(self, closure=None):
        if closure is not None:
            raise RuntimeError("DeviceAdamW.step() takes no closure: the gradients are read from the flat buffer")
        self._upload_hyper()
        self._enqueue(self._amp_word("grad_scale"), self._amp_word("found_inf"))
        _ops.bump_weights_epoch()

    def zero_grad(self, set_to_none=True):
        self.buckets.zero_grad()

    def state_dict(self):
        sd = super().state_dict()
        steps = self._state[0].expand(len(sd["state"])).clone().unbind(0)
        sd["state"] = {k: {**ent, "step": s} for (k, ent), s in zip(sd["state"].items(), steps)}
        return sd

    @torch.no_grad()
    def load_state_dict(self, state_dict):
        groups = state_dict["param_groups"]
        if len(groups) != 1 or len(groups[0]["params"]) != len(self.buckets.params):
            raise ValueError("DeviceAdamW.load_state_dict: expected one param group over %d parameters" % len(self.buckets.params))
        src, state = groups[0], state_dict["state"]
        if src.get("amsgrad") or src.get("maximize"):
            raise ValueError("DeviceAdamW.load_state_dict: amsgrad / maximize states cannot be continued here")
        if len(state) not in (0, len(self.buckets.params)):
            raise ValueError("DeviceAdamW.load_state_dict: state for %d of %d parameters" % (len(state), len(self.buckets.params)))
        steps = set()
        for key, p in zip(src["params"], self.buckets.params):
            ent = state.get(key)
            if ent is None:
                continue
            if tuple(ent["exp_avg"].shape) != tuple(p.shape) or tuple(ent["exp_avg_sq"].shape) != tuple(p.shape):
                raise ValueError("DeviceAdamW.load_state_dict: moment shapes do not match the parameters")
            steps.add(float(ent["step"]))
        if len(steps) > 1:
            raise ValueError(f"DeviceAdamW.load_state_dict: the parameters carry different step counts {sorted(steps)}; "
                             "one flat update has one step count")
        for key, p in zip(src["params"], self.buckets.params):
            ent = state.get(key)
            mine = self.state[p]
            if ent is None:
                mine["exp_avg"].zero_(); mine["exp_avg_sq"].zero_()
            else:
                if ent["exp_avg"].data_ptr() != mine["exp_avg"].data_ptr():
                    mine["exp_avg"].copy_(ent["exp_avg"])
                if ent["exp_avg_sq"].data_ptr() != mine["exp_avg_sq"].data_ptr():
                    mine["exp_avg_sq"].copy_(ent["exp_avg_sq"])
        self._state[0].fill_(steps.pop() if steps else 0.0)
        group = self.param_groups[0]
        for k, val in src.items():
            if k != "params":
                group[k] = val
        group.setdefault("max_norm", self.defaults["max_norm"])
        self._hyper_host = None
```

### include/hriemo.h

```cpp
#ifndef HRIEMO_H_
#define HRIEMO_H_

#ifdef __cplusplus
extern "C" {
#endif

typedef struct ihipStream_t* hriemo_stream_t;

const char* hriemo_last_error(void);
int hriemo_abi_version(void);

int hriemo_gemm_bf16(int ta, int tb, int M, int N, int K, const void* A, long lda, const void* B, long ldb,
                     void* C, long ldc, int c_is_f32, const float* bias, int epilogue, const void* aux,
                     long ldaux, int accumulate, float* workspace, long workspace_bytes, hriemo_stream_t stream);

int hriemo_gemm_bf16_group_tn(const void* jobs_host, int njobs, int accumulate, hriemo_stream_t stream);
int hriemo_gemm_bf16_split(int ta, int tb, int M, int N, int K, const void* A, long lda, const void* B, long ldb, void* C, long ldc,
                           void* C2, long ldc2, int split_m, int accumulate, float* workspace, long workspace_bytes,
                           hriemo_stream_t stream);
int hriemo_gemm_colsum_rows(int ta, int tb, int M, int N, int K);
int hriemo_gemm_bf16_colsum(int ta, int tb, int M, int N, int K, const void* A, long lda, const void* B, long ldb, void* C, long ldc,
                            const void* aux, long ldaux, float* colsum_partials, hriemo_stream_t stream);
int hriemo_gemm_force_config(int cfg);
int hriemo_gemm_debug_flags(int flags);
// ... 91 lines not shown
int hriemo_add_ln_bwd(const void* dY, const void* G, const void* X, const float* X32, const float* gamma, const float* mean,
                      const float* rstd, void* dX, void* dG, float* dgamma, float* dbeta, float* dbias, int accumulate,
                      int M, int d, float p_drop, unsigned long long seed, const unsigned long long* seed_dev,
                      unsigned site, long row_offset, float* workspace, hriemo_stream_t stream);

long hriemo_colsum_workspace_bytes(int M, int N);
int hriemo_colsum_bf16(const void* X, long ldx, int M, int N, float* out, int accumulate, float* workspace,
                       hriemo_stream_t stream);
int hriemo_cast_f32_to_bf16(const float* src, void* dst, long n, hriemo_stream_t stream);
int hriemo_cast_bf16_to_f32(const void* src, float* dst, long n, hriemo_stream_t stream);
int hriemo_cast_f32_to_bf16_batch(const void* jobs_host, int njobs, hriemo_stream_t stream);
int hriemo_cast_copy_batch(const void* jobs_host, int njobs, hriemo_stream_t stream);
int hriemo_dropout_bf16(const void* X, void* Y, long M, int N, float p_drop, unsigned long long seed,
                        const unsigned long long* seed_dev, unsigned site, long row_offset, hriemo_stream_t stream);
int hriemo_expand_rows(const float* q, void* out, float* out32, int B, long n, hriemo_stream_t stream);
int hriemo_seed_bump(unsigned long long* seed_dev, hriemo_stream_t stream);
int hriemo_rowdot_fwd(const void* Z, const float* Z32, const float* w, const float* b, float* out, int M, int d,
                      hriemo_stream_t stream);
int hriemo_rowdot_bwd(const float* dl, const void* Z, const float* Z32, const float* w, void* dZ, float* dw, float* db, int accumulate,
                      int M, int d, hriemo_stream_t stream);

int hriemo_pool_chunks(int L);
int hriemo_ln_pool_fwd(const void* X, const float* X32, const unsigned char* mask, const float* gamma, const float* beta, void* Yn,
                       float* mean, float* rstd, float* partials, int B, int L, int Lkeep, int d, float eps,
                       hriemo_stream_t stream);
int hriemo_gate_input(const float* partials_a, const float* partials_t, const unsigned char* mask_a,
                      const unsigned char* mask_t, int B, int La, int Lt, int d, void* gate_in, float* a_pool,
                      float* t_pool, float* cnt, hriemo_stream_t stream);
int hriemo_sigmoid_beta(const float* pre, float* w, float* beta, int B, int d, hriemo_stream_t stream);
int hriemo_fuse_fwd(const float* w, const void* A, const void* T, void* H, int B, int L, int d, hriemo_stream_t stream);
int hriemo_fuse_bwd_dw(const void* dH, const void* A, const void* T, float* partials, int B, int L, int d,
                       hriemo_stream_t stream);
int hriemo_gate_dpre(const float* partials, int L, const float* dbeta, const float* w, void* dpre, int B, int d,
                     hriemo_stream_t stream);
int hriemo_gate_input_bwd(const void* dgin, const float* a_pool, const float* t_pool, const float* cnt, float* da,
                          float* dt, int B, int d, hriemo_stream_t stream);
int hriemo_masked_mean_fwd(const void* X, const unsigned char* mask, float* pooled, float* cnt, int B, int L, int d,
                           hriemo_stream_t stream);
int hriemo_rowsum_f32(const float* x, float* out, int B, long n, hriemo_stream_t stream);
int hriemo_gate_input_pooled(const float* a_pool, const float* t_pool, void* gate_in, int B, int d, hriemo_stream_t stream);
int hriemo_fusion_loss(const float* logits, const float* targets, const float* pos_weight, const float* beta, int B, int Ne,
                       int reg_mode, float reg_coef, float scale, float* loss, float* dlogits, float* dbeta, hriemo_stream_t stream);
int hriemo_fusion_loss_ce(const float* logits, const long long* labels, const float* beta, int B, int C, int reg_mode,
                          float reg_coef, float scale, float* loss, float* dlogits, float* dbeta, hriemo_stream_t stream);
int hriemo_fusion_loss_n(const float* logits, const float* targets, const float* pos_weight, const float* beta, int B, int Ne,
                         int reg_mode, float reg_coef, float scale, float* loss, float* dlogits, float* dbeta, const int* n_valid,
                         hriemo_stream_t stream);
int hriemo_fusion_loss_ce_n(const float* logits, const long long* labels, const float* beta, int B, int C, int reg_mode,
                            float reg_coef, float scale, float* loss, float* dlogits, float* dbeta, const int* n_valid,
                            hriemo_stream_t stream);
int hriemo_stats_update(const float* logits, const float* targets, const long long* labels, const float* loss, float loss_scale,
                        const float* beta, int beta_per_sample, const int* n_valid, int B, int C, int skip_nonfinite,
                        float* probs, unsigned char* truth, int capacity, int* counters, double* sums, hriemo_stream_t stream);
int hriemo_stats_counts(const float* probs, const unsigned char* truth, int capacity, int C, const int* counters,
                        const float* thresholds, int S, int* out, hriemo_stream_t stream);
int hriemo_stats_auc_tiles(int capacity);
int hriemo_stats_auc(const float* probs, const unsigned char* truth, int capacity, int C, const int* counters,
                     unsigned long long* partial, int* npn, hriemo_stream_t stream);
int hriemo_predict_log(const float* logits, const float* beta, int beta_per_sample, const int* n_valid, int B, int C, int kind,
                       float* probs, float* beta_mean, int* pred, int capacity, int* counters, hriemo_stream_t stream);
int hriemo_attn_log_plan(const int* lens, const int* n_valid, int B, int capacity, int* counters, int* window, int* lengths,
                         hriemo_stream_t stream);
int hriemo_attn_log_close(int* window, hriemo_stream_t stream);
int hriemo_attn_log_append(const float* maps, int B, int map_elems, const int* window, float* log, int capacity,
                           hriemo_stream_t stream);
int hriemo_attn_probs_varlen_log(const void* Q, long ldq, const void* K, long ldk, const int* cu_seqlens_q, const int* cu_seqlens_k,
                                 const float* lse, float* probs, int B, int H, int max_len_q, int max_len_k, int out_lq, int out_lk,
                                 int head_dim, float p_drop, unsigned long long seed, const unsigned long long* seed_dev, unsigned site,
                                 int b_offset, const int* window, int capacity, hriemo_stream_t stream);
int hriemo_attn_probs_varlen_log_fp32(const float* Q, long ldq, const float* K, long ldk, const int* cu_seqlens_q,
                                     const int* cu_seqlens_k, const float* lse, float* probs, int B, int H, int max_len_q, int max_len_k,
                                     int out_lq, int out_lk, int head_dim, float p_drop, unsigned long long seed,
                                     const unsigned long long* seed_dev, unsigned site, int b_offset, const int* window, int capacity,
                                     hriemo_stream_t stream);
int hriemo_scalar_gate_dx(const void* dH, int Lf, const float* beta, int is_a, const float* dpool, const float* cnt,
                          const unsigned char* mask, void* dX, int B, int L, int d, hriemo_stream_t stream);
int hriemo_sumsq_f32(const float* x, long n, float* partial, int nblocks, hriemo_stream_t stream);
int hriemo_adamw_flat(float* p, const float* g, float* m, float* v, long n, float lr, float beta1, float beta2, float eps,
                      float weight_decay, int step, float max_norm, const float* norm2, hriemo_stream_t stream);
int hriemo_optim_finalize(const float* partial, int nblocks, const float* hyper, const float* grad_scale, const float* found_inf,
                          float* state, hriemo_stream_t stream);
int hriemo_adamw_flat_dev(float* p, const float* g, float* m, float* v, long n, const float* hyper, const float* state,
                          hriemo_stream_t stream);
int hriemo_grad_begin(float* flat, long n, const int* ctl, hriemo_stream_t stream);
int hriemo_optim_finalize_ctl(const float* partial, int nblocks, const float* hyper, const float* grad_scale, const float* found_inf,
                              float* state, const int* ctl, hriemo_stream_t stream);
int hriemo_add_ln_bwd_partial_rows(int M, int d);
int hriemo_rowops_force_variant(int variant);
int hriemo_colsum_partial_rows(int M, int N);
int hriemo_colreduce_batch(const void* jobs_host, int njobs, void* jobs_dev, int nblocks, hriemo_stream_t stream);
int hriemo_debug_hog(int blocks, int micros, float* sink, hriemo_stream_t stream);
int hriemo_ln_pool_pair_supported(int d);
int hriemo_ln_pool_fwd_pair(const void* Xa, const float* Xa32, const unsigned char* mask_a, const float* gamma_a, const float* beta_a,
                            void* Yna, float* mean_a, float* rstd_a, float* partials_a, int La,
                            const void* Xt, const float* Xt32, const unsigned char* mask_t, const float* gamma_t, const float* beta_t,
                            void* Ynt, float* mean_t, float* rstd_t, float* partials_t, int Lt,
                            int B, int Lkeep, int d, float eps, hriemo_stream_t stream);
int hriemo_ln_pool_bwd_pair(const void* dH, int Lf, const float* w,
                            const float* dpool_a, const unsigned char* mask_a, const void* Xa, const float* Xa32, const float* gamma_a,
                            const float* mean_a, const float* rstd_a, void* dXa, float* dgamma_a, float* dbeta_a, int La, float* workspace_a,
                            const float* dpool_t, const unsigned char* mask_t, const void* Xt, const float* Xt32, const float* gamma_t,
                            const float* mean_t, const float* rstd_t, void* dXt, float* dgamma_t, float* dbeta_t, int Lt, float* workspace_t,
                            int accumulate, int B, int d, hriemo_stream_t stream);
int hriemo_ln_pool_bwd_chunks(int L);
long hriemo_ln_pool_bwd_workspace_bytes(int B, int L, int d);
int hriemo_ln_pool_bwd(const void* dH, int Lf, const float* w, int is_a, const float* dpool, const unsigned char* mask,
                       const void* X, const float* X32, const float* gamma, const float* mean, const float* rstd, void* dX,
                       float* dgamma, float* dbeta, int accumulate, int B, int L, int d, float* workspace, hriemo_stream_t stream);

int hriemo_ln_pool_fwd_packed(const void* X, const float* X32, const int* cu_seqlens, int nseq, int n_rows, const float* gamma,
                              const float* beta, void* Yn, float* mean, float* rstd, float* partials, int L,
                              const int* cu_fused, int n_fused, int B, int d, float eps, hriemo_stream_t stream);
int hriemo_ln_pool_fwd_packed_pair(const void* Xa, const float* Xa32, const int* cu_a, int nseq_a, int n_rows_a, const float* gamma_a,
                                   const float* beta_a, void* Yna, float* mean_a, float* rstd_a, float* partials_a, int La,
                                   const void* Xt, const float* Xt32, const int* cu_t, int nseq_t, int n_rows_t, const float* gamma_t,
                                   const float* beta_t, void* Ynt, float* mean_t, float* rstd_t, float* partials_t, int Lt,
                                   const int* cu_fused, int n_fused, int B, int d, float eps, hriemo_stream_t stream);
int hriemo_fuse_fwd_packed(const float* w, const void* A, const void* T, void* H, const int* cu_fused, int n_fused, int B, int L, int d,
                           hriemo_stream_t stream);
int hriemo_fuse_fwd_packed_q(const float* w, const void* A, const void* T, void* H, const int* cu_fused, int n_fused, int B, int L, int d,
                             void* Hq, void* Hs, long lds, hriemo_stream_t stream);
int hriemo_fuse_bwd_dw_packed(const void* dH, const void* A, const void* T, float* partials, const int* cu_fused, int n_fused, int B,
                              int L, int d, hriemo_stream_t stream);
int hriemo_ln_pool_bwd_packed(const void* dH, const int* cu_fused, int n_fused, const float* w, int is_a, const float* dpool,
                              const void* X, const float* X32, const int* cu_seqlens, int nseq, int n_rows, const float* gamma,
                              const float* mean, const float* rstd, void* dX, float* dgamma, float* dbeta, int accumulate, int B, int L,
                              int d, float* workspace, hriemo_stream_t stream);
int hriemo_ln_pool_bwd_packed_pair(const void* dH, const int* cu_fused, int n_fused, const float* w,
                                   const float* dpool_a, const void* Xa, const float* Xa32, const int* cu_a, int nseq_a, int n_rows_a,
                                   const float* gamma_a, const float* mean_a, const float* rstd_a, void* dXa, float* dgamma_a,
                                   float* dbeta_a, int La, float* workspace_a,
                                   const float* dpool_t, const void* Xt, const float* Xt32, const int* cu_t, int nseq_t, int n_rows_t,
                                   const float* gamma_t, const float* mean_t, const float* rstd_t, void* dXt, float* dgamma_t,
                                   float* dbeta_t, int Lt, float* workspace_t, int accumulate, int B, int d, hriemo_stream_t stream);

int hriemo_split_bf16x3(const float* X, long ldx, int M, int K, void* Y, int layout, int relu, hriemo_stream_t stream);
int hriemo_attn_fwd_f32(const float* Q, long ldq, const float* K, long ldk, const float* V, long ldv, float* O, long ldo,
                        const unsigned char* key_padding_mask, float* lse, int B, int H, int Lq, int Lk, int head_dim,
                        float p_drop, unsigned long long seed, const unsigned long long* seed_dev, unsigned site, int b_offset,
                        hriemo_stream_t stream);
int hriemo_attn_probs_f32(const float* Q, long ldq, const float* K, long ldk, const unsigned char* key_padding_mask,
                          const float* lse, float* probs, int B, int H, int Lq, int Lk, int head_dim, float p_drop,
                          unsigned long long seed, const unsigned long long* seed_dev, unsigned site, int b_offset,
                          hriemo_stream_t stream);
int hriemo_add_ln_f32(const float* G, const float* X, const float* gamma, const float* beta, float* Y32, void* Y16, int M, int d,
                      float eps, float p_drop, unsigned long long seed, const unsigned long long* seed_dev, unsigned site,
                      long row_offset, hriemo_stream_t stream);
int hriemo_dropout_f32(const float* X, float* Y, long M, int N, int relu, const float* gate, float p_drop, unsigned long long seed,
                       const unsigned long long* seed_dev, unsigned site, long row_offset, hriemo_stream_t stream);
int hriemo_masked_mean_f32(const float* X, const unsigned char* mask, float* pooled, int B, int L, int d, hriemo_stream_t stream);
int hriemo_gate_input_f32(const float* a_pool, const float* t_pool, float* gate_in, int B, int d, hriemo_stream_t stream);
int hriemo_sigmoid_beta_f32(const float* pre, float* w, float* beta, int B, int d, hriemo_stream_t stream);
int hriemo_fuse_f32(const float* w, const float* A, int La, const float* T, int Lt, float* H32, void* H16, int B, int L, int d,
                    hriemo_stream_t stream);

int hriemo_split3_f32(const float* X, long ldx, int M, int K, void* Y, int form, int relu, const float* mask, long ldmask,
                      hriemo_stream_t stream);
long hriemo_colsum_f32_workspace_bytes(int M, int N);
int hriemo_colsum_f32(const float* X, long ldx, int M, int N, const float* mask, long ldmask, float* out, int accumulate,
                      float* workspace, hriemo_stream_t stream);
long hriemo_add_ln_bwd_f32_workspace_bytes(int M, int d);
int hriemo_add_ln_bwd_f32(const float* dY, const float* G, const float* X, const float* gamma, float* dS, float* dG, float* dgamma,
                          float* dbeta, float* dbias, int accumulate, int M, int d, float eps, float p_drop, unsigned long long seed,
                          const unsigned long long* seed_dev, unsigned site, long row_offset, float* workspace, hriemo_stream_t stream);
int hriemo_attn_bwd_f32(const float* Q, long ldq, const float* K, long ldk, const float* V, long ldv, const float* O, long ldo,
                        const float* dO, long lddo, const unsigned char* key_padding_mask, const float* lse, float* dQ, long lddq,
// ... 59 lines not shown
```

Before: 8748 utterances/s.

## Write bf16 weight shadows from the AdamW kernel and drop per-step recasts

```diff
diff --git a/hri-emo_amd/__init__.py b/hri-emo_amd/__init__.py
--- a/hri-emo_amd/__init__.py
+++ b/hri-emo_amd/__init__.py
@@ -7,7 +7,7 @@
 from .models.fusion_classifier import FusionClassifier
 
 from .dp import EvalStep
-from ._ops import set_gemm_mode, gemm_mode, enable_fused_wgrad, set_precision, precision, set_varlen, varlen, set_varlen_maps, varlen_maps, set_mfma_maps, mfma_maps, set_ingest, ingest
+from ._ops import set_gemm_mode, gemm_mode, enable_fused_wgrad, set_precision, precision, set_varlen, varlen, set_varlen_maps, varlen_maps, set_mfma_maps, mfma_maps, set_ingest, ingest, set_step_prelude, step_prelude
 
-__all__ = ["EvalStep", "set_gemm_mode", "gemm_mode", "enable_fused_wgrad", "set_precision", "precision", "set_varlen", "varlen", "set_varlen_maps", "varlen_maps", "set_mfma_maps", "mfma_maps", "set_ingest", "ingest", "CrossModalBlock", "CrossModalTransformer", "BetaGate", "EmotionDecoder", "ExplainableDecoderLayer",
+__all__ = ["EvalStep", "set_gemm_mode", "gemm_mode", "enable_fused_wgrad", "set_precision", "precision", "set_varlen", "varlen", "set_varlen_maps", "varlen_maps", "set_mfma_maps", "mfma_maps", "set_ingest", "ingest", "set_step_prelude", "step_prelude", "CrossModalBlock", "CrossModalTransformer", "BetaGate", "EmotionDecoder", "ExplainableDecoderLayer",
            "FusionWithEmotionDecoder", "MoseiFusionWithEmotionDecoder", "FusionClassifier"]
diff --git a/hri-emo_amd/_lib.py b/hri-emo_amd/_lib.py
--- a/hri-emo_amd/_lib.py
+++ b/hri-emo_amd/_lib.py
@@ -103,6 +103,8 @@
     "hriemo_adamw_flat": ("pppplfffffifpp", "i"),
     "hriemo_optim_finalize": ("pippppp", "i"),
     "hriemo_adamw_flat_dev": ("pppplppp", "i"),
+    "hriemo_adamw_flat_shadow": ("pppplfffffifppip", "i"),
+    "hriemo_adamw_flat_dev_shadow": ("pppplpppip", "i"),
     "hriemo_grad_begin": ("plpp", "i"),
     "hriemo_optim_finalize_ctl": ("pipppppp", "i"),
     "hriemo_masked_mean_fwd": ("ppppiiip", "i"),
diff --git a/hri-emo_amd/_ops.py b/hri-emo_amd/_ops.py
--- a/hri-emo_amd/_ops.py
+++ b/hri-emo_amd/_ops.py
@@ -208,16 +208,74 @@
     return int(torch.randint(0, 2 ** 62, (1,)).item())
 
 
+PRELUDE_PARTS = ("casts", "copies")
+_PRELUDE_LEGACY = None
+
+
+def set_step_prelude(value):
+    global _PRELUDE_LEGACY
+    parts = set()
+    for word in (value or "").replace(" ", "").split(","):
+        if word == "":
+            continue
+        if word == "legacy":
+            parts.update(PRELUDE_PARTS)
+        elif word.startswith("legacy:") and word[7:] in PRELUDE_PARTS:
+            parts.add(word[7:])
+        else:
+            raise ValueError(f"step prelude {value!r}: '', 'legacy' or a comma list of " + ", ".join("legacy:" + q for q in PRELUDE_PARTS))
+    _PRELUDE_LEGACY = frozenset(parts)
+
+
+def step_prelude():
+    if _PRELUDE_LEGACY is None:
+        set_step_prelude(_os.environ.get("HRIEMO_STEP_PRELUDE", ""))
+    if _PRELUDE_LEGACY == frozenset(PRELUDE_PARTS):
+        return "legacy"
+    return ",".join("legacy:" + q for q in PRELUDE_PARTS if q in _PRELUDE_LEGACY)
+
+
+def prelude_legacy(part):
+    if _PRELUDE_LEGACY is None:
+        set_step_prelude(_os.environ.get("HRIEMO_STEP_PRELUDE", ""))
+    return part in _PRELUDE_LEGACY
+
+
+def _pver(p):
+    flat = getattr(p, "_hriemo_flat", None)
+    return (p._version, p.data_ptr(), -1 if flat is None else flat._version)
+
+
 class Shadows:
 
     def __init__(self):
         self._d = {}
+        self._reg = {}
+
+    def _register(self, key, parts):
+        ok = True
+        for p, e0, n, dst, d0, kind in parts:
+            if not p.is_contiguous() or (p.data_ptr() + e0 * 4) % 16 or (dst.data_ptr() + d0 * dst.element_size()) % 16:
+                ok = False
+        if ok:
+            self._reg[key] = parts
+        else:
+            self._reg.pop(key, None)
+
+    def _managed(self, key, ent):
+        return ent is not None and key in self._reg and not prelude_legacy("casts")
+
+    def _key_version(self, key):
+        parts = self._reg[key]
+        if isinstance(key, int):
+            return _pver(parts[0][0]) + (WEIGHTS_EPOCH,)
+        return tuple(_pver(p) for p, *_ in parts) + (WEIGHTS_EPOCH,)
 
     def get(self, p):
         key = id(p)
         ent = self._d.get(key)
-        ver = (p._version, p.data_ptr(), WEIGHTS_EPOCH)
-        if (CTX.capturing and (ent is None or len(ent) < 3 or ent[2] != STEP_ID)) or ent is None or ent[0] != ver or ent[1].device != p.device:
+        ver = _pver(p) + (WEIGHTS_EPOCH,)
+        if (CTX.capturing and not self._managed(key, ent) and (ent is None or len(ent) < 3 or ent[2] != STEP_ID)) or ent is None or ent[0] != ver or ent[1].device != p.device:
             s = ent[1] if ent is not None and ent[1].device == p.device and ent[1].shape == p.shape else \
                 torch.empty(p.shape, dtype=BF16, device=p.device)
             _require_gpu(p)
@@ -228,6 +286,7 @@
             _lib.call("hriemo_cast_f32_to_bf16", _p(src), _p(s), src.numel(), _stream())
             ent = (ver, s, STEP_ID)
             self._d[key] = ent
+            self._register(key, [(p, 0, p.numel(), s, 0, 0)])
         return ent[1]
 
     def prefetch(self, params):
@@ -236,21 +295,21 @@
 
     def stale(self, p):
         ent = self._d.get(id(p))
-        ver = (p._version, p.data_ptr(), WEIGHTS_EPOCH)
-        need = (CTX.capturing and (ent is None or len(ent) < 3 or ent[2] != STEP_ID)) or ent is None or ent[0] != ver or ent[1].device != p.device
+        ver = _pver(p) + (WEIGHTS_EPOCH,)
+        need = (CTX.capturing and not self._managed(id(p), ent) and (ent is None or len(ent) < 3 or ent[2] != STEP_ID)) or ent is None or ent[0] != ver or ent[1].device != p.device
         dst = ent[1] if ent is not None and ent[1].device == p.device and ent[1].shape == p.shape else None
         return need, dst, ver
 
     def get_cat(self, parts):
         key = ("cat",) + tuple((id(p), r0, r1) for p, r0, r1 in parts)
         ent = self._d.get(key)
-        ver = tuple((p._version, p.data_ptr()) for p, _, _ in parts) + (WEIGHTS_EPOCH,)
+        ver = tuple(_pver(p) for p, _, _ in parts) + (WEIGHTS_EPOCH,)
         dev = parts[0][0].device
-        if (CTX.capturing and (ent is None or ent[2] != STEP_ID)) or ent is None or ent[0] != ver or ent[1].device != dev:
+        if (CTX.capturing and not self._managed(key, ent) and (ent is None or ent[2] != STEP_ID)) or ent is None or ent[0] != ver or ent[1].device != dev:
             rows = sum(r1 - r0 for _, r0, r1 in parts)
             K = parts[0][0].shape[1]
             s = ent[1] if ent is not None and ent[1].device == dev else torch.empty((rows, K), dtype=BF16, device=dev)
-            at = 0
+            at, reg = 0, []
             for p, r0, r1 in parts:
                 _require_gpu(p)
                 _require_fp32_master(p)
@@ -258,20 +317,22 @@
                 if not src.is_contiguous():
                     src = src.contiguous()
                 _lib.call("hriemo_cast_f32_to_bf16", _p(src[r0:r1]), _p(s[at:at + (r1 - r0)]), (r1 - r0) * K, _stream())
+                reg.append((p, r0 * K, (r1 - r0) * K, s, at * K, 0))
                 at += r1 - r0
             ent = (ver, s, STEP_ID)
             self._d[key] = ent
+            self._register(key, reg)
         return ent[1]
 
     def get_cat_wb(self, wparts, bparts):
         kw = ("cat",) + tuple((id(p), r0, r1) for p, r0, r1 in wparts)
         kb = ("catv",) + tuple((id(p), r0, r1) for p, r0, r1 in bparts)
         ew, eb = self._d.get(kw), self._d.get(kb)
-        vw = tuple((p._version, p.data_ptr()) for p, _, _ in wparts) + (WEIGHTS_EPOCH,)
-        vb = tuple((p._version, p.data_ptr()) for p, _, _ in bparts) + (WEIGHTS_EPOCH,)
+        vw = tuple(_pver(p) for p, _, _ in wparts) + (WEIGHTS_EPOCH,)
+        vb = tuple(_pver(p) for p, _, _ in bparts) + (WEIGHTS_EPOCH,)
         dev = wparts[0][0].device
-        stale_w = (CTX.capturing and (ew is None or ew[2] != STEP_ID)) or ew is None or ew[0] != vw or ew[1].device != dev
-        stale_b = (CTX.capturing and (eb is None or eb[2] != STEP_ID)) or eb is None or eb[0] != vb or eb[1].device != dev
+        stale_w = (CTX.capturing and not self._managed(kw, ew) and (ew is None or ew[2] != STEP_ID)) or ew is None or ew[0] != vw or ew[1].device != dev
+        stale_b = (CTX.capturing and not self._managed(kb, eb) and (eb is None or eb[2] != STEP_ID)) or eb is None or eb[0] != vb or eb[1].device != dev
         if not (stale_w or stale_b):
             return ew[1], eb[1]
         if not all(p.is_contiguous() for p, _, _ in wparts + bparts):
@@ -281,16 +342,18 @@
         nb = sum(r1 - r0 for _, r0, r1 in bparts)
         sw = ew[1] if ew is not None and ew[1].device == dev and ew[1].shape == (rows, K) else torch.empty((rows, K), dtype=BF16, device=dev)
         sb = eb[1] if eb is not None and eb[1].device == dev and eb[1].shape == (nb,) else torch.empty((nb,), dtype=torch.float32, device=dev)
-        jobs, at = [], 0
+        jobs, at, regw, regb = [], 0, [], []
         for p, r0, r1 in wparts:
             _require_gpu(p)
             _require_fp32_master(p)
             jobs.append((p.data_ptr() + r0 * K * 4, sw.data_ptr() + at * K * 2, (r1 - r0) * K, 0))
+            regw.append((p, r0 * K, (r1 - r0) * K, sw, at * K, 0))
             at += r1 - r0
         at = 0
         for p, r0, r1 in bparts:
             _require_fp32_master(p)
             jobs.append((p.data_ptr() + r0 * 4, sb.data_ptr() + at * 4, r1 - r0, 1))
+            regb.append((p, r0, r1 - r0, sb, at, 1))
             at += r1 - r0
         if any(j[0] % 16 or j[1] % 16 for j in jobs):
             return self.get_cat(wparts), self.get_cat_vec(bparts)
@@ -298,12 +361,14 @@
         _lib.call("hriemo_cast_copy_batch", host.data_ptr(), len(jobs), _stream())
         self._d[kw] = (vw, sw, STEP_ID)
         self._d[kb] = (vb, sb, STEP_ID)
+        self._register(kw, regw)
+        self._register(kb, regb)
         return sw, sb
 
     def get_cat_mx8(self, parts):
         key = ("catmx",) + tuple((id(p), r0, r1) for p, r0, r1 in parts)
         ent = self._d.get(key)
-        ver = tuple((p._version, p.data_ptr()) for p, _, _ in parts) + (WEIGHTS_EPOCH,)
+        ver = tuple(_pver(p) for p, _, _ in parts) + (WEIGHTS_EPOCH,)
         if CTX.capturing or ent is None or ent[0] != ver:
             rows = sum(r1 - r0 for _, r0, r1 in parts)
             K = parts[0][0].shape[1]
@@ -333,15 +398,48 @@
     def get_cat_vec(self, parts):
         key = ("catv",) + tuple((id(p), r0, r1) for p, r0, r1 in parts)
         ent = self._d.get(key)
-        ver = tuple((p._version, p.data_ptr()) for p, _, _ in parts) + (WEIGHTS_EPOCH,)
-        if (CTX.capturing and (ent is None or ent[2] != STEP_ID)) or ent is None or ent[0] != ver:
+        ver = tuple(_pver(p) for p, _, _ in parts) + (WEIGHTS_EPOCH,)
+        if (CTX.capturing and not self._managed(key, ent) and (ent is None or ent[2] != STEP_ID)) or ent is None or ent[0] != ver:
             v = torch.cat([p.detach()[r0:r1] for p, r0, r1 in parts])
             if ent is not None and ent[1].shape == v.shape and ent[1].device == v.device:
                 ent[1].copy_(v)
                 v = ent[1]
             ent = (ver, v, STEP_ID)
             self._d[key] = ent
+            reg, at = [], 0
+            for p, r0, r1 in parts:
+                reg.append((p, r0, r1 - r0, v, at, 1))
+                at += r1 - r0
+            self._register(key, reg)
         return ent[1]
+
+    def _current(self, key):
+        ent = self._d.get(key)
+        return ent is not None and ent[0] == self._key_version(key) and all(ent[1] is q[3] for q in self._reg[key])
+
+    def _mark_current(self, key):
+        ent = self._d[key]
+        self._d[key] = (self._key_version(key),) + tuple(ent[1:])
+
+    def stale_jobs(self):
+        jobs, keys = [], []
+        for key, parts in self._reg.items():
+            ent = self._d.get(key)
+            if ent is None or not all(ent[1] is q[3] for q in parts):
+                continue
+            if ent[0] == self._key_version(key):
+                continue
+            if any(p.numel() < e0 + n for p, e0, n, dst, d0, kind in parts):
+                raise RuntimeError("a weight changed its size behind a captured step: capture the step again")
+            if any((p.data_ptr() + e0 * 4) % 16 or p.device != dst.device or p.dtype != torch.float32 or not p.is_contiguous()
+                   for p, e0, n, dst, d0, kind in parts):
+                for p, e0, n, dst, d0, kind in parts:
+                    dst.view(-1)[d0:d0 + n].copy_(p.detach().reshape(-1)[e0:e0 + n])
+                self._mark_current(key)
+                continue
+            jobs += [(p.data_ptr() + e0 * 4, dst.data_ptr() + d0 * dst.element_size(), n, kind) for p, e0, n, dst, d0, kind in parts]
+            keys.append(key)
+        return jobs, keys
 
 
 FUSED_WGRAD = True
@@ -402,12 +500,85 @@
         if dst is None:
             dst = torch.empty(p.shape, dtype=BF16, device=p.device)
         jobs.append((p.data_ptr(), dst.data_ptr(), p.numel()))
-        upd.append((sh, id(p), ver, dst))
+        upd.append((sh, p, ver, dst))
     if jobs:
         host = torch.tensor(jobs, dtype=torch.int64)
         _lib.call("hriemo_cast_f32_to_bf16_batch", host.data_ptr(), len(jobs), _stream())
-        for sh, key, ver, dst in upd:
-            sh._d[key] = (ver, dst, STEP_ID)
+        for sh, p, ver, dst in upd:
+            sh._d[id(p)] = (ver, dst, STEP_ID)
+            sh._register(id(p), [(p, 0, p.numel(), dst, 0, 0)])
+
+
+def model_shadows(model):
+    return [m._sh for m in model.modules() if isinstance(getattr(m, "_sh", None), Shadows)]
+
+
+def sync_shadows(shadows):
+    jobs, marks = [], []
+    for sh in shadows:
+        j, keys = sh.stale_jobs()
+        jobs += j
+        marks += [(sh, k) for k in keys]
+    if jobs:
+        host = torch.tensor(jobs, dtype=torch.int64)
+        _lib.call("hriemo_cast_copy_batch", host.data_ptr(), len(jobs), _stream())
+        for sh, k in marks:
+            sh._mark_current(k)
+    return len(jobs)
+
+
+class ShadowMap:
+
+    def __init__(self, shadows, buckets, flat_p):
+        rows, self.covered, self.held = [], [], []
+        base = flat_p.data_ptr()
+        for sh in shadows:
+            for key, parts in sh._reg.items():
+                ent = sh._d.get(key)
+                if ent is None or not all(ent[1] is q[3] for q in parts):
+                    continue
+                mine = []
+                for p, e0, n, dst, d0, kind in parts:
+                    off = buckets._offsets.get(id(p))
+                    if off is None or p.data_ptr() != base + off * 4 or dst.device != flat_p.device or p.numel() < e0 + n or dst.numel() < d0 + n:
+                        break
+                    mine.append((off + e0, n, dst.data_ptr() + d0 * dst.element_size(), kind))
+                else:
+                    rows += mine
+                    self.covered.append((sh, key))
+                    self.held.append((ent[1], [(q[0], buckets._offsets[id(q[0])]) for q in parts]))
+        self.table, self.nrec = shadow_map_table(rows, flat_p.device)
+        self.flat_ptr = base
+        self.signature = tuple(sorted(rows))
+
+    def valid_for(self, flat_p):
+        if self.nrec == 0 or flat_p.data_ptr() != self.flat_ptr:
+            return False
+        for (sh, key), (dst, homes) in zip(self.covered, self.held):
+            ent = sh._d.get(key)
+            if ent is None or ent[1] is not dst or any(p.data_ptr() != self.flat_ptr + off * 4 for p, off in homes):
+                return False
+        return True
+
+    def current(self):
+        return [(sh, key) for sh, key in self.covered if key in sh._reg and sh._current(key)]
+
+
+def shadow_map_table(rows, device):
+    rows = sorted(rows)
+    reach, top = [], 0
+    for first, n, _, _ in rows:
+        top = max(top, first + n)
+        reach.append(top)
+    words = [w for r in rows for w in r] + reach
+    table = torch.tensor(words if words else [0], dtype=torch.int64).to(device)
+    return table, len(rows)
+
+
+def weights_updated_with(current):
+    bump_weights_epoch()
+    for sh, key in current:
+        sh._mark_current(key)
 
 
 def padded_shadow(sh, p, kp):
diff --git a/hri-emo_amd/csrc/common.h b/hri-emo_amd/csrc/common.h
--- a/hri-emo_amd/csrc/common.h
+++ b/hri-emo_amd/csrc/common.h
@@ -125,3 +125,45 @@
   for (int i = 0; i < 8; ++i) v[i] = (bf16_t)f[i];
   return v;
 }
+
+__device__ __forceinline__ int shadow_first_record(const long long* __restrict__ map, int nrec, long e0) {
+  const long long* reach = map + 4 * (long)nrec;
+  int lo = 0, hi = nrec;
+  while (lo < hi) {
+    const int mid = (lo + hi) >> 1;
+    if (reach[mid] > e0) hi = mid; else lo = mid + 1;
+  }
+  return lo;
+}
+__device__ __forceinline__ void shadow_store4(const long long* __restrict__ map, int nrec, int j0, long span_end, long e, const f32x4& pp) {
+  for (int j = j0; j < nrec; ++j) {
+    const long first = (long)map[4 * j];
+    if (first >= span_end) break;
+    const long end = first + (long)map[4 * j + 1];
+    if (first >= e + 4 || end <= e) continue;
+    const long o = e - first;
+    const bool whole = o >= 0 && e + 4 <= end;
+    if (map[4 * j + 3] != 0) {
+      float* d = (float*)map[4 * j + 2];
+      if (whole && ((uintptr_t)(d + o) & 15) == 0) {
+        *(f32x4*)(d + o) = pp;
+      } else {
+#pragma unroll
+        for (int k = 0; k < 4; ++k)
+          if (e + k >= first && e + k < end) d[o + k] = pp[k];
+      }
+    } else {
+      bf16_t* d = (bf16_t*)map[4 * j + 2];
+      if (whole && ((uintptr_t)(d + o) & 7) == 0) {
+        bf16x4 h;
+#pragma unroll
+        for (int k = 0; k < 4; ++k) h[k] = (bf16_t)pp[k];
+        *(bf16x4*)(d + o) = h;
+      } else {
+#pragma unroll
+        for (int k = 0; k < 4; ++k)
+          if (e + k >= first && e + k < end) d[o + k] = (bf16_t)pp[k];
+      }
+    }
+  }
+}
diff --git a/hri-emo_amd/csrc/optim.hip b/hri-emo_amd/csrc/optim.hip
--- a/hri-emo_amd/csrc/optim.hip
+++ b/hri-emo_amd/csrc/optim.hip
@@ -43,9 +43,10 @@
   state[ST_DECAY] = 1.f - lr * wd;
 }
 
+template <bool SHADOW>
 __global__ __launch_bounds__(256) void adamw_flat_dev_kernel(float* __restrict__ p, const float* __restrict__ g, float* __restrict__ m,
                                                              float* __restrict__ v, long n, const float* __restrict__ hyper,
-                                                             const float* __restrict__ state) {
+                                                             const float* __restrict__ state, const long long* __restrict__ map, int nrec) {
   if (state[ST_SKIP] != 0.f) return;
   const float b1 = hyper[HY_BETA1], b2 = hyper[HY_BETA2], eps = hyper[HY_EPS];
   const float coef = state[ST_COEF], step = state[ST_STEP_SIZE], isb2 = state[ST_ISB2], decay = state[ST_DECAY];
@@ -61,6 +62,10 @@
       pp[e] -= step * mm[e] / (sqrtf(vv[e]) * isb2 + eps);
     }
     *(f32x4*)(p + i * 4) = pp; *(f32x4*)(m + i * 4) = mm; *(f32x4*)(v + i * 4) = vv;
+    if (SHADOW) {
+      const long span = (i - threadIdx.x) * 4;
+      shadow_store4(map, nrec, shadow_first_record(map, nrec, span), span + 1024, i * 4, pp);
+    }
   }
 }
 
@@ -102,15 +107,30 @@
   return 0;
 }
 
-extern "C" int hriemo_adamw_flat_dev(float* p, const float* g, float* m, float* v, long n, const float* hyper, const float* state,
-                                     hipStream_t st) {
+static int adamw_flat_dev_launch(float* p, const float* g, float* m, float* v, long n, const float* hyper, const float* state,
+                                 const void* shadow_map, int nrec, hipStream_t st) {
   HRIEMO_CHECK(n > 0 && n % 4 == 0, "adamw_flat_dev: n=%ld must be a positive multiple of 4", n);
   HRIEMO_CHECK(((uintptr_t)p % 16) == 0 && ((uintptr_t)g % 16) == 0 && ((uintptr_t)m % 16) == 0 && ((uintptr_t)v % 16) == 0,
                "adamw_flat_dev: unaligned buffer");
   HRIEMO_CHECK(hyper != nullptr && state != nullptr, "adamw_flat_dev: hyper and state are required");
   long gsz = (n / 4 + 255) / 256;
   if (gsz > 4096) gsz = 4096;
-  hipLaunchKernelGGL(adamw_flat_dev_kernel, dim3((int)gsz), dim3(256), 0, st, p, g, m, v, n, hyper, state);
+  if (nrec > 0)
+    hipLaunchKernelGGL(adamw_flat_dev_kernel<true>, dim3((int)gsz), dim3(256), 0, st, p, g, m, v, n, hyper, state, (const long long*)shadow_map, nrec);
+  else
+    hipLaunchKernelGGL(adamw_flat_dev_kernel<false>, dim3((int)gsz), dim3(256), 0, st, p, g, m, v, n, hyper, state, (const long long*)nullptr, 0);
   HRIEMO_LAUNCH_CHECK("adamw_flat_dev_kernel");
   return 0;
 }
+
+extern "C" int hriemo_adamw_flat_dev(float* p, const float* g, float* m, float* v, long n, const float* hyper, const float* state,
+                                     hipStream_t st) {
+  return adamw_flat_dev_launch(p, g, m, v, n, hyper, state, nullptr, 0, st);
+}
+
+extern "C" int hriemo_adamw_flat_dev_shadow(float* p, const float* g, float* m, float* v, long n, const float* hyper, const float* state,
+                                            const void* shadow_map, int nrec, hipStream_t st) {
+  HRIEMO_CHECK(nrec >= 0 && (nrec == 0 || (shadow_map != nullptr && ((uintptr_t)shadow_map % 8) == 0)),
+               "adamw_flat_dev_shadow: nrec=%d records need an 8-byte aligned map in device memory", nrec);
+  return adamw_flat_dev_launch(p, g, m, v, n, hyper, state, shadow_map, nrec, st);
+}
diff --git a/hri-emo_amd/csrc/rowops.hip b/hri-emo_amd/csrc/rowops.hip
--- a/hri-emo_amd/csrc/rowops.hip
+++ b/hri-emo_amd/csrc/rowops.hip
@@ -1347,10 +1347,24 @@
   HRIEMO_LAUNCH_CHECK("cast_f32_bf16_kernel");
   return 0;
 }
-struct CastJobs { const float* src[64]; void* dst[64]; long n[64]; int first[65]; int njobs; unsigned long long f32_copy; };
+typedef __attribute__((ext_vector_type(4))) unsigned u32x4c;
+struct CastJobs { const float* src[64]; void* dst[64]; long n[64]; int first[65]; int njobs; unsigned long long f32_copy, byte_copy; };
+#define BYTE_JOB_SPAN 16384
 __global__ __launch_bounds__(256) void cast_f32_bf16_batch_kernel(const CastJobs J) {
   int j = 0;
   while (j + 1 < J.njobs && (int)blockIdx.x >= J.first[j + 1]) ++j;
+  if ((J.byte_copy >> j) & 1ull) {
+    const char* s = (const char*)J.src[j];
+    char* d = (char*)J.dst[j];
+    const long nb = J.n[j], b0 = ((long)blockIdx.x - J.first[j]) * BYTE_JOB_SPAN + (long)threadIdx.x * 16;
+#pragma unroll
+    for (int u = 0; u < BYTE_JOB_SPAN / 4096; ++u) {
+      const long o = b0 + u * 4096;
+      if (o + 16 <= nb) *(u32x4c*)(d + o) = *(const u32x4c*)(s + o);
+      else for (long e = o; e < nb; ++e) d[e] = s[e];
+    }
+    return;
+  }
   const long n = J.n[j], base = ((long)blockIdx.x - J.first[j]) * 2048 + (long)threadIdx.x * 8;
   const float* src = J.src[j];
   if ((J.f32_copy >> j) & 1ull) {
@@ -1377,15 +1391,20 @@
     CastJobs J;
     const int nj = njobs - j0 < 64 ? njobs - j0 : 64;
     int blocks = 0;
-    J.f32_copy = 0ull;
+    J.f32_copy = J.byte_copy = 0ull;
     for (int j = 0; j < nj; ++j) {
       const long long* r = h + (long)(j0 + j) * rec;
       HRIEMO_CHECK(r[2] > 0 && (r[0] % 16) == 0 && (r[1] % 16) == 0, "cast_batch: job %d empty or unaligned", j0 + j);
-      HRIEMO_CHECK(rec == 3 || r[3] == 0 || r[3] == 1, "cast_batch: job %d has kind %lld (0 = fp32 -> bf16, 1 = fp32 copy)", j0 + j, r[3]);
+      HRIEMO_CHECK(rec == 3 || (r[3] >= 0 && r[3] <= 2), "cast_batch: job %d has kind %lld (0 = fp32 -> bf16, 1 = fp32 copy, 2 = byte copy)",
+                   j0 + j, r[3]);
+      const bool bytes = rec == 4 && r[3] == 2;
+      const long long nblk = bytes ? (r[2] + BYTE_JOB_SPAN - 1) / BYTE_JOB_SPAN : (r[2] + 2047) / 2048;
+      HRIEMO_CHECK(nblk + blocks <= 0x7fffffffll, "cast_batch: job %d makes the grid too large", j0 + j);
       J.src[j] = (const float*)r[0]; J.dst[j] = (void*)r[1]; J.n[j] = (long)r[2];
       if (rec == 4 && r[3] == 1) J.f32_copy |= 1ull << j;
+      if (bytes) J.byte_copy |= 1ull << j;
       J.first[j] = blocks;
-      blocks += (int)((r[2] + 2047) / 2048);
+      blocks += (int)nblk;
     }
     J.first[nj] = blocks; J.njobs = nj;
     hriemo_prof_begin(HP_ROWOPS, st);
@@ -1826,9 +1845,11 @@
   if (threadIdx.x == 0) partial[blockIdx.x] = red[0] + red[1] + red[2] + red[3];
 }
 
+template <bool SHADOW>
 __global__ __launch_bounds__(256) void adamw_flat_kernel(float* __restrict__ p, const float* __restrict__ g, float* __restrict__ m,
                                                          float* __restrict__ v, long n, float lr, float b1, float b2, float eps,
-                                                         float wd, float bc1, float bc2, float max_norm, const float* __restrict__ norm2) {
+                                                         float wd, float bc1, float bc2, float max_norm, const float* __restrict__ norm2,
+                                                         const long long* __restrict__ map, int nrec) {
   float coef = 1.f;
   if (max_norm > 0.f) coef = fminf(1.f, max_norm / (sqrtf(norm2[0]) + 1e-6f));
   const float step = lr / bc1, isb2 = 1.f / sqrtf(bc2);
@@ -1844,6 +1865,10 @@
       pp[e] -= step * mm[e] / (sqrtf(vv[e]) * isb2 + eps);
     }
     *(f32x4*)(p + i * 4) = pp; *(f32x4*)(m + i * 4) = mm; *(f32x4*)(v + i * 4) = vv;
+    if (SHADOW) {
+      const long span = (i - threadIdx.x) * 4;
+      shadow_store4(map, nrec, shadow_first_record(map, nrec, span), span + 1024, i * 4, pp);
+    }
   }
 }
 
@@ -1952,18 +1977,35 @@
   return 0;
 }
 
-extern "C" int hriemo_adamw_flat(float* p, const float* g, float* m, float* v, long n, float lr, float beta1, float beta2, float eps,
-                                 float weight_decay, int step, float max_norm, const float* norm2, hipStream_t st) {
+static int adamw_flat_launch(float* p, const float* g, float* m, float* v, long n, float lr, float beta1, float beta2, float eps,
+                             float weight_decay, int step, float max_norm, const float* norm2, const void* shadow_map, int nrec, hipStream_t st) {
   HRIEMO_CHECK(n > 0 && n % 4 == 0 && step >= 1, "adamw_flat: n=%ld must be a positive multiple of 4 and step >= 1", n);
   HRIEMO_CHECK(((uintptr_t)p % 16) == 0 && ((uintptr_t)g % 16) == 0 && ((uintptr_t)m % 16) == 0 && ((uintptr_t)v % 16) == 0, "adamw_flat: unaligned buffer");
   HRIEMO_CHECK(max_norm <= 0.f || norm2 != nullptr, "adamw_flat: clipping needs the squared gradient norm");
   const float bc1 = 1.f - powf(beta1, (float)step), bc2 = 1.f - powf(beta2, (float)step);
   long gsz = (n / 4 + 255) / 256;
   if (gsz > 4096) gsz = 4096;
-  hipLaunchKernelGGL(adamw_flat_kernel, dim3((int)gsz), dim3(256), 0, st, p, g, m, v, n, lr, beta1, beta2, eps, weight_decay, bc1, bc2,
-                     max_norm, norm2);
+  if (nrec > 0)
+    hipLaunchKernelGGL(adamw_flat_kernel<true>, dim3((int)gsz), dim3(256), 0, st, p, g, m, v, n, lr, beta1, beta2, eps, weight_decay, bc1, bc2,
+                       max_norm, norm2, (const long long*)shadow_map, nrec);
+  else
+    hipLaunchKernelGGL(adamw_flat_kernel<false>, dim3((int)gsz), dim3(256), 0, st, p, g, m, v, n, lr, beta1, beta2, eps, weight_decay, bc1, bc2,
+                       max_norm, norm2, (const long long*)nullptr, 0);
   HRIEMO_LAUNCH_CHECK("adamw_flat_kernel");
   return 0;
+}
+
+extern "C" int hriemo_adamw_flat(float* p, const float* g, float* m, float* v, long n, float lr, float beta1, float beta2, float eps,
+                                 float weight_decay, int step, float max_norm, const float* norm2, hipStream_t st) {
+  return adamw_flat_launch(p, g, m, v, n, lr, beta1, beta2, eps, weight_decay, step, max_norm, norm2, nullptr, 0, st);
+}
+
+extern "C" int hriemo_adamw_flat_shadow(float* p, const float* g, float* m, float* v, long n, float lr, float beta1, float beta2, float eps,
+                                        float weight_decay, int step, float max_norm, const float* norm2, const void* shadow_map, int nrec,
+                                        hipStream_t st) {
+  HRIEMO_CHECK(nrec >= 0 && (nrec == 0 || (shadow_map != nullptr && ((uintptr_t)shadow_map % 8) == 0)),
+               "adamw_flat_shadow: nrec=%d records need an 8-byte aligned map in device memory", nrec);
+  return adamw_flat_launch(p, g, m, v, n, lr, beta1, beta2, eps, weight_decay, step, max_norm, norm2, shadow_map, nrec, st);
 }
 
 extern "C" int hriemo_fuse_fwd(const float* w, const void* A, const void* T, void* H, int B, int L, int d, hipStream_t st) {
diff --git a/hri-emo_amd/dp.py b/hri-emo_amd/dp.py
--- a/hri-emo_amd/dp.py
+++ b/hri-emo_amd/dp.py
@@ -250,14 +250,18 @@
 
 
 class _GraphRecord:
-    __slots__ = ("graph", "loss", "keep", "seqs", "out")
+    __slots__ = ("graph", "loss", "keep", "seqs", "out", "sync_shadows", "shadow_map", "in_sync")
 
     def __init__(self, graph, loss, keep, seqs=None, out=None):
         self.graph, self.loss, self.keep, self.seqs, self.out = graph, loss, keep, seqs, out
+        self.sync_shadows = False
+        self.shadow_map = None
+        self.in_sync = []
 
     def release(self):
         from . import _ops
-        self.graph = self.loss = self.keep = self.seqs = self.out = None
+        self.graph = self.loss = self.keep = self.seqs = self.out = self.shadow_map = None
+        self.in_sync = []
         _ops.GRAPHS_ALIVE -= 1
         if _ops.GRAPHS_ALIVE == 0:
             del _ops._ws_retired[:]
@@ -417,7 +421,36 @@
     _ops.GRAPHS_ALIVE += 1
     keep = _ops._deferred.keep + _ops._small_dw.keep
     _ops._deferred.keep, _ops._small_dw.keep = [], []
-    return _GraphRecord(graph, out, keep, seqs)
+    rec = _GraphRecord(graph, out, keep, seqs)
+    rec.sync_shadows = not _ops.prelude_legacy("casts")
+    return rec
+
+
+def _hand_over(pairs):
+    from . import _lib, _ops
+    jobs = []
+    for s, t in pairs:
+        raw = (not _ops.prelude_legacy("copies") and t.dtype == s.dtype and t.device == s.device and t.shape == s.shape and s.numel() > 0
+               and t.is_contiguous() and s.is_contiguous() and s.data_ptr() % 16 == 0 and t.data_ptr() % 16 == 0)
+        if raw:
+            jobs.append((t.data_ptr(), s.data_ptr(), s.numel() * s.element_size(), 2))
+        else:
+            s.copy_(t)
+    if jobs:
+        host = torch.tensor(jobs, dtype=torch.int64)
+        _lib.call("hriemo_cast_copy_batch", host.data_ptr(), len(jobs), _ops._stream())
+
+
+def _replay(rec, owner):
+    from . import _ops
+    if rec.sync_shadows:
+        sh = owner.__dict__.get("_shadows")
+        if sh is None:
+            sh = owner._shadows = _ops.model_shadows(owner.model)
+        _ops.sync_shadows(sh)
+    if rec.shadow_map is not None:
+        rec.in_sync = rec.shadow_map.current()
+    rec.graph.replay()
 
 
 class DataParallelStep:
@@ -445,6 +478,7 @@
         self._stats_scale = 1.0
         self._outputs = None
         self._feed = None
+        self._graph_map = None
 
     @property
     def captured(self):
@@ -689,10 +723,10 @@
             self._optimizer._upload_hyper()
         key = load((first, last))
         rec = self._packed_graph(key)
-        rec.graph.replay()
+        _replay(rec, self)
         self._micro = 0 if last else self._micro + 1
         if last:
-            self._after_replay()
+            self._after_replay(rec)
         return rec.loss
 
     def _eager_ragged(self, rows_a, rows_t, la, lt, y):
@@ -777,6 +811,7 @@
 
         def warmed():
             self._outputs = None
+            self._leave_shadow_map()
 
         def body():
             _ops.bump_seed_word(self._static[0].device)
@@ -787,13 +822,28 @@
             if self._optimizer is not None:
                 front = self._pb.front if self._pb is not None else None
                 ctl = front.ctl.dev if (front is not None and front.accum > 1) else None
-                self._optimizer._enqueue(ctl=ctl)
+                smap = self._optimizer._enqueue(ctl=ctl)
+                self._graph_map = smap
             return loss
 
         if seqs is not None and self._pb.pool is None:
             self._pb.pool = torch.cuda.graph_pool_handle()
-        return _record_graph(self._static[0].device, seqs, self._pb.pool if seqs is not None else None, warm, body, warmed,
-                             settle=0.25 if collectives else 0.0)
+        self._graph_map = None
+        rec = _record_graph(self._static[0].device, seqs, self._pb.pool if seqs is not None else None, warm, body, warmed,
+                            settle=0.25 if collectives else 0.0)
+        rec.shadow_map = self._graph_map
+        return rec
+
+    def _leave_shadow_map(self):
+        from . import _ops
+        b = self.buckets
+        flat_p = getattr(b.params[0], "_hriemo_flat", None) if b.params else None
+        if _ops.prelude_legacy("casts") or flat_p is None:
+            return
+        smap = _ops.ShadowMap(_ops.model_shadows(self.model), b, flat_p)
+        old = getattr(b, "shadow_map", None)
+        if old is None or old.signature != smap.signature or not old.valid_for(flat_p):
+            b.shadow_map = smap if smap.nrec else None
 
     def release_graph(self):
         if self.captured:
@@ -809,12 +859,12 @@
         self._replay = bool(on) and self.captured
         self.buckets.suspended = self._replay
 
-    def _after_replay(self):
+    def _after_replay(self, rec=None):
         if not self._exchange_in_graph:
             self.buckets.finish()
         if self._optimizer is not None:
             from . import _ops
-            _ops.bump_weights_epoch()
+            _ops.weights_updated_with(rec.in_sync if rec is not None else [])
             self._optimizer._opt_called = True
 
     @_in_step_context
@@ -837,12 +887,11 @@
                 else:
                     key = self._packed_key(m_a, m_t, lengths)
                     self._mask_seen = _MaskSeen(ident, key, (pb.cu_a.clone(), pb.cu_t.clone(), pb.cu_f.clone()), (m_a, m_t))
-            for s, t in zip(self._static, (h_a, h_t, m_a, m_t, y)):
-                if s is not None and t is not None and s.data_ptr() != t.data_ptr():
-                    s.copy_(t)
+            _hand_over([(s, t) for s, t in zip(self._static, (h_a, h_t, m_a, m_t, y))
+                        if s is not None and t is not None and s.data_ptr() != t.data_ptr()])
             rec = self._packed_graph(key) if pb is not None else self._record
-            rec.graph.replay()
-            self._after_replay()
+            _replay(rec, self)
+            self._after_replay(rec)
             return rec.loss
         loss = self._fwd_bwd(h_a, h_t, m_a, m_t, y)
         self._update_stats()
@@ -991,7 +1040,7 @@
             return self._eval_eager(rows_a, rows_t, la, lt, y if targets else None)
         self._check_modes("eval_store", "capture_store")
         rec = self._packed_graph(_load_ragged(pb, self._static, feed.fill(ids, targets), la, lt))
-        rec.graph.replay()
+        _replay(rec, self)
         logits, beta, z = rec.out
         n = len(ids)
         return logits[:n], beta[:n], z[:n], rec.loss
@@ -1083,7 +1132,7 @@
                 raise ValueError(f"eval_packed: targets of shape {tuple(y.shape)}; captured with {tuple(sy.shape)}"
                                  + (f", this batch needs {want}" if n != pb.B else ""))
         rec = self._packed_graph(_load_ragged(pb, self._static, _caller_rows(rows_a, rows_t, y), la, lt))
-        rec.graph.replay()
+        _replay(rec, self)
         logits, beta, z = rec.out
         return logits[:n], beta[:n], z[:n], rec.loss
 
diff --git a/hri-emo_amd/optim.py b/hri-emo_amd/optim.py
--- a/hri-emo_amd/optim.py
+++ b/hri-emo_amd/optim.py
@@ -20,6 +20,7 @@
                 view = self.flat_p[off:off + n].view_as(p)
                 view.copy_(p.data)
                 p.data = view
+                p._hriemo_flat = self.flat_p
         self.nblocks = 1024
         self._partial = torch.empty(self.nblocks, dtype=torch.float32, device=flat_g.device)
         self._norm2 = torch.zeros(1, dtype=torch.float32, device=flat_g.device)
@@ -33,10 +34,25 @@
         self.steps += 1
         _lib.call("hriemo_sumsq_f32", _p(g), n, _p(self._partial), self.nblocks, st)
         _lib.call("hriemo_rowsum_f32", _p(self._partial), _p(self._norm2), 1, self.nblocks, st)
-        _lib.call("hriemo_adamw_flat", _p(self.flat_p), _p(g), _p(self.m), _p(self.v), n, self.lr, self.betas[0], self.betas[1],
-                  self.eps, self.wd, self.steps, self.max_norm if self.max_norm else 0.0, _p(self._norm2), st)
-        _ops.bump_weights_epoch()
+        smap = _shadow_map(self.buckets, self.flat_p)
+        if smap is None:
+            _lib.call("hriemo_adamw_flat", _p(self.flat_p), _p(g), _p(self.m), _p(self.v), n, self.lr, self.betas[0], self.betas[1],
+                      self.eps, self.wd, self.steps, self.max_norm if self.max_norm else 0.0, _p(self._norm2), st)
+            _ops.bump_weights_epoch()
+        else:
+            current = smap.current()
+            _lib.call("hriemo_adamw_flat_shadow", _p(self.flat_p), _p(g), _p(self.m), _p(self.v), n, self.lr, self.betas[0],
+                      self.betas[1], self.eps, self.wd, self.steps, self.max_norm if self.max_norm else 0.0, _p(self._norm2),
+                      _p(smap.table), smap.nrec, st)
+            _ops.weights_updated_with(current)
         return self._norm2.sqrt()
+
+
+def _shadow_map(buckets, flat_p):
+    smap = getattr(buckets, "shadow_map", None)
+    if smap is None or _ops.prelude_legacy("casts") or not smap.valid_for(flat_p):
+        return None
+    return smap
 
 
 class DeviceAdamW(torch.optim.Optimizer):
@@ -67,6 +83,7 @@
                 view = self.flat_p[off:off + n].view_as(p)
                 view.copy_(p.data)
                 p.data = view
+                p._hriemo_flat = self.flat_p
                 self.state[p] = {"step": self._state[0], "exp_avg": self.m[off:off + n].view_as(p),
                                  "exp_avg_sq": self.v[off:off + n].view_as(p)}
         self.grad_norm, self.device_step, self.skipped = self._state[6], self._state[0], self._state[7]
@@ -98,7 +115,13 @@
         else:
             _lib.call("hriemo_optim_finalize_ctl", _p(self._partial), self.nblocks, _p(self._hyper), _p(grad_scale), _p(found_inf),
                       _p(self._state), _p(ctl), st)
-        _lib.call("hriemo_adamw_flat_dev", _p(self.flat_p), _p(g), _p(self.m), _p(self.v), n, _p(self._hyper), _p(self._state), st)
+        smap = _shadow_map(self.buckets, self.flat_p) if ctl is None else None
+        if smap is None:
+            _lib.call("hriemo_adamw_flat_dev", _p(self.flat_p), _p(g), _p(self.m), _p(self.v), n, _p(self._hyper), _p(self._state), st)
+        else:
+            _lib.call("hriemo_adamw_flat_dev_shadow", _p(self.flat_p), _p(g), _p(self.m), _p(self.v), n, _p(self._hyper), _p(self._state),
+                      _p(smap.table), smap.nrec, st)
+        return smap
 
     def _amp_word(self, name):
         t = getattr(self, name, None)
@@ -113,8 +136,10 @@
         if closure is not None:
             raise RuntimeError("DeviceAdamW.step() takes no closure: the gradients are read from the flat buffer")
         self._upload_hyper()
+        smap = _shadow_map(self.buckets, self.flat_p)
+        current = smap.current() if smap is not None else []
         self._enqueue(self._amp_word("grad_scale"), self._amp_word("found_inf"))
-        _ops.bump_weights_epoch()
+        _ops.weights_updated_with(current)
 
     def zero_grad(self, set_to_none=True):
         self.buckets.zero_grad()
diff --git a/include/hriemo.h b/include/hriemo.h
--- a/include/hriemo.h
+++ b/include/hriemo.h
@@ -197,6 +197,11 @@
                           float* state, hriemo_stream_t stream);
 int hriemo_adamw_flat_dev(float* p, const float* g, float* m, float* v, long n, const float* hyper, const float* state,
                           hriemo_stream_t stream);
+int hriemo_adamw_flat_shadow(float* p, const float* g, float* m, float* v, long n, float lr, float beta1, float beta2, float eps,
+                             float weight_decay, int step, float max_norm, const float* norm2, const void* shadow_map, int nrec,
+                             hriemo_stream_t stream);
+int hriemo_adamw_flat_dev_shadow(float* p, const float* g, float* m, float* v, long n, const float* hyper, const float* state,
+                                 const void* shadow_map, int nrec, hriemo_stream_t stream);
 int hriemo_grad_begin(float* flat, long n, const int* ctl, hriemo_stream_t stream);
 int hriemo_optim_finalize_ctl(const float* partial, int nblocks, const float* hyper, const float* grad_scale, const float* found_inf,
                               float* state, const int* ctl, hriemo_stream_t stream);
diff --git a/scripts_dev/ab_step_prelude.py b/scripts_dev/ab_step_prelude.py
--- /dev/null
+++ b/scripts_dev/ab_step_prelude.py
@@ -0,0 +1,130 @@
+import os
+import statistics
+import sys
+import time
+
+import torch
+
+sys.path.insert(0, os.path.dirname(os.path.dirname(os.path.abspath(__file__))))
+import hri_emo_amd as H
+from hri_emo_amd import _ops
+from hri_emo_amd.dp import DataParallelStep
+from hri_emo_amd.optim import FusedClipAdamW
+from hri_emo_amd.train import fusion_step_loss
+import bench
+
+args = sys.argv[1:]
+UPDATE = "--update" in args
+args = [a for a in args if a != "--update"]
+ROUNDS = int(args[0]) if len(args) > 0 else 7
+STEPS = int(args[1]) if len(args) > 1 else 30
+ARMS = [("legacy", "legacy"), ("new", ""), ("casts-only", "legacy:copies"), ("copies-only", "legacy:casts")]
+dev = torch.device("cuda", 0)
+wl = bench.WORKLOADS["cfg2"]
+bench.CFG = dict(wl["model"], beta_hidden=256, dropout=0.1)
+bench.T_A, bench.T_T = wl["T_a"], wl["T_t"]
+H.set_gemm_mode(wl["gemm"])
+B = wl["batch"]
+
+
+def report(res, names):
+    med = {}
+    for name in names:
+        r = res[name]
+        med[name] = statistics.median(r)
+        print(f"  {name:12s} median {med[name]:.4f} ms  spread (max - min) {max(r) - min(r):.4f} ms  (" + " ".join(f"{x:.4f}" for x in r) + ")", flush=True)
+    spread = max(res["legacy"]) - min(res["legacy"])
+    for name in names:
+        if name == "legacy":
+            continue
+        d = med["legacy"] - med[name]
+        verdict = "faster" if d > 3 * spread else ("SLOWER" if -d > 3 * spread else "no gain beyond the noise")
+        print(f"  legacy - {name:12s} = {d:+.4f} ms ({100 * d / med['legacy']:+.2f} %); 3 x legacy's spread = {3 * spread:.4f} ms -> {verdict}", flush=True)
+
+
+def evaluation(Bv):
+    from hri_emo_amd import data
+    g = torch.Generator().manual_seed(100)
+    smp = []
+    for _ in range(Bv):
+        la = int(torch.randint(int(0.44 * bench.T_A), bench.T_A + 1, (1,), generator=g))
+        lt = int(torch.randint(int(0.44 * bench.T_T), bench.T_T + 1, (1,), generator=g))
+        smp.append((torch.randn(la, 768, generator=g), torch.zeros(la, dtype=torch.bool), torch.randn(lt, 768, generator=g),
+                    torch.zeros(lt, dtype=torch.bool), (torch.rand(6, generator=g) < 0.3).float()))
+    r_a, l_a, r_t, l_t, y = data.collate_seq_packed(smp)
+    rag = (r_a.bfloat16().to(dev), r_t.bfloat16().to(dev), l_a.tolist(), l_t.tolist(), y.to(dev))
+    arms = {}
+    for name, prelude in ARMS[:2]:
+        _ops.set_step_prelude(prelude)
+        torch.manual_seed(1234)
+        model = H.FusionWithEmotionDecoder(**bench.CFG).to(dev).train()
+        es = H.EvalStep(model, fusion_step_loss)
+        es.capture_packed(*rag, pad_to=(bench.T_A, bench.T_T))
+        arms[name] = es
+    s_a, s_t = sum(rag[2]), sum(rag[3])
+    res = {name: [] for name in arms}
+    for rnd in range(ROUNDS):
+        for name in (list(arms) if rnd % 2 == 0 else list(arms)[::-1]):
+            es = arms[name]
+            st = es._static
+            run = lambda: es.eval_packed(st[0][:s_a], st[1][:s_t], rag[2], rag[3], st[4])
+            for _ in range(3):
+                run()
+            torch.cuda.synchronize()
+            t0 = time.perf_counter()
+            for _ in range(STEPS):
+                run()
+            torch.cuda.synchronize()
+            res[name].append((time.perf_counter() - t0) / STEPS * 1e3)
+    print(f"EvalStep replay, B = {Bv}, inputs resident:")
+    report(res, list(arms))
+    for es in arms.values():
+        es.release_graph()
+
+
+def main():
+    print(f"ab_step_prelude: rounds {ROUNDS}, replays per round {STEPS}, optimizer step per replay: {UPDATE}, {torch.cuda.get_device_name(0)}")
+    steps = {}
+    for name, prelude in ARMS:
+        _ops.set_step_prelude(prelude)
+        torch.manual_seed(1234)
+        model = H.FusionWithEmotionDecoder(**bench.CFG).to(dev).train()
+        dp = DataParallelStep(model, fusion_step_loss, overlap=False)
+        opt = FusedClipAdamW(dp.buckets, lr=1e-4, weight_decay=1e-2, max_norm=5.0)
+        dp.set_global_batch(B)
+        batch = bench.synth(B, 0, dev)
+        dp.step(*batch)
+        dp.capture(*batch)
+        steps[name] = (prelude, dp, opt, batch)
+    res = {name: [] for name, _ in ARMS}
+    for rnd in range(ROUNDS):
+        for name, _ in (ARMS if rnd % 2 == 0 else ARMS[::-1]):
+            prelude, dp, opt, batch = steps[name]
+            _ops.set_step_prelude(prelude)
+            for _ in range(3):
+                dp.step(*batch)
+                if UPDATE:
+                    opt.step()
+            torch.cuda.synchronize()
+            t0 = time.perf_counter()
+            for _ in range(STEPS):
+                dp.step(*batch)
+                if UPDATE:
+                    opt.step()
+            torch.cuda.synchronize()
+            res[name].append((time.perf_counter() - t0) / STEPS * 1e3)
+    print("the captured train step (cfg 2, B = 64):")
+    report(res, [name for name, _ in ARMS])
+    for _, dp, _, _ in steps.values():
+        dp.release_graph()
+    del steps
+    if not UPDATE:
+        H.set_varlen(True)
+        H.set_ingest(True)
+        _ops.PACKED_TAIL = True
+        for Bv in (64, 8):
+            evaluation(Bv)
+
+
+if __name__ == "__main__":
+    main()
```

Result: no change. 8823 utterances/s, median of 6 (+0.9%).
